# jinsungkim96/MPC-SensorlessAO

Hardware: AMD Instinct MI355X
Metric: MPC steps/sec (n=27, VAR(2), T=30) (higher is better)
Workload: dtype f64

## Files before the change

mpc-sensorlessao_amd/csrc/fmpc_affine.h:

```cpp
#pragma once
#include <hip/hip_runtime.h>
#include "fmpc_host.h"
#include "../../include/fastmpc.h"

#define FA_N 27

struct FaStep {
    const double* x0; const double* x0p; const double* nu0;
    double* zout; double* nuout; double* u0out; int* status; int* iters; double* step;
    int* need;
};

struct FaParams {
    int n, m, T, nb, has_xf, batch, rows, tiles, step_ld;
    int nu_rows, nu_tiles;
    int ldz;
    int tiles_used, wgs_per_group;
    const double* img;
    const double* imgE; const double* imgEp;
    const double* elin; const double* eplin;
    const double* dx0T;
    double e0, ep0, normE, norme, normEp, normep, rd2_0;
    const double* x0; const double* x0p; const double* nu0;
    double* zout; double* nuout; double* u0out; int* status; int* iters; double* step;
    int* need; int* handed;
    int* nflag;
    double* dump;
    int nsteps;
    FaStep steps[FMPC_STRETCH_MAX];
    int nlanes, wgs_per_lane;
    int lane_begin[FMPC_STRETCH_MAX + 1];
    const double* imgG;
    const int* plan;
    int jbase, nu_work;
    int nparts, nitems, swap;
};

#define FMPC_STRETCH_LANES_DEFAULT FMPC_STRETCH_MAX
hipError_t fmpc_launch_affine(FaParams P, int num_cu, hipStream_t stream, const unsigned* supersedes = nullptr);
hipError_t fmpc_launch_affine_nu(FaParams P, int grid, bool nt, hipStream_t stream);
```

mpc-sensorlessao_amd/csrc/fmpc_api.hip:

```cpp
#include <hip/hip_runtime.h>
#include <math.h>
#include <stdio.h>
#include <stdlib.h>
#include <string.h>
#include <atomic>
#include <map>
#include <mutex>
#include <new>
#include <vector>

#include "../../include/fastmpc.h"
#include "fmpc_device.h"
#include "fmpc_panel.h"
#include "fmpc_host.h"
#include "fmpc_first.h"
#include "fmpc_affine.h"
#include "fmpc_loopu0.h"
#include "fmpc_tiled.h"
#include "fmpc_rampcold.h"
#include "fmpc_bank.h"
#include "fmpc_records.h"
#include "fmpc_kkt.h"
#include "fmpc_estimator.h"
#include "fmpc_handle.h"
// ... 603 lines not shown
bool fmpc_capturing(hipStream_t stream) {
    hipStreamCaptureStatus st = hipStreamCaptureStatusNone;
    return hipStreamIsCapturing(stream, &st) == hipSuccess && st == hipStreamCaptureStatusActive;
}

struct FmpcChainStep {
    FaStep a;
    FwParams w;
    bool superseded;
    unsigned same_outputs;
};
struct FmpcStretch {
    fmpc_handle h = nullptr;
    int nsteps = 0;
    FaParams A;
    double k = 0.0; int n_newton = 0, zld = 0, g3 = 0; bool z_null = false, z_aligned = false;
    size_t wave_lds = 0, ws_stride = 0; int num_cu = 0;
    FwParams* table = nullptr;
    FmpcChainStep st[FMPC_STRETCH_MAX];
    size_t nodes_seen = 0;
};
static std::mutex fmpc_st_mu;
static std::map<hipStream_t, FmpcStretch> fmpc_st_map;
static std::atomic<int> fmpc_st_open{0};

static bool fmpc_capture_nodes(hipStream_t stream, size_t* count) {
    hipStreamCaptureStatus st = hipStreamCaptureStatusNone;
    unsigned long long id = 0; hipGraph_t graph = nullptr; const hipGraphNode_t* deps = nullptr; size_t ndeps = 0;
    if (hipStreamGetCaptureInfo_v2(stream, &st, &id, &graph, &deps, &ndeps) != hipSuccess || st != hipStreamCaptureStatusActive || !graph)
        return false;
    size_t n = 0;
    if (hipGraphGetNodes(graph, nullptr, &n) != hipSuccess) return false;
    *count = n;
    return true;
}
static void fmpc_stretch_look(FmpcStretch& S, hipStream_t stream) {
    size_t n = 0;
    S.nodes_seen = fmpc_capture_nodes(stream, &n) ? n : 0;
}
static bool fmpc_stretch_foreign(FmpcStretch& S, hipStream_t stream) {
    size_t n = 0;
    if (S.nsteps == 0 || !fmpc_capture_nodes(stream, &n) || n == S.nodes_seen) return false;
    S.nsteps = 0; S.h = nullptr;
    S.nodes_seen = n;
    return true;
}

static int fmpc_stretch_flush(FmpcStretch& S, hipStream_t stream) {
    if (S.nsteps == 0) return FMPC_OK;
    const int n = S.nsteps;
    fmpc_handle h = S.h;
    S.nsteps = 0; S.h = nullptr;
    if (!fmpc_capturing(stream) && h->ev && h->ev_valid && h->last_stream != stream && hipStreamWaitEvent(stream, h->ev, 0) != hipSuccess)
        return FMPC_E_HIP;
    FaParams A = S.A;
    A.nsteps = n;
    for (int i = 0; i < n; ++i) A.steps[i] = S.st[i].a;
    unsigned same[FMPC_STRETCH_MAX];
    for (int j = 0; j < n; ++j) {
        same[j] = S.st[j].same_outputs & ((1u << j) - 1u);
        for (int i = 0; i < j; ++i) if (same[j] >> i & 1u) same[j] |= same[i];
    }
    if (fmpc_launch_affine(A, S.num_cu, stream, same) != hipSuccess) return FMPC_E_HIP;
    int live[FMPC_STRETCH_MAX], nlive = 0;
    for (int i = 0; i < n; ++i) if (!S.st[i].superseded) live[nlive++] = i;
    int launches = 1;
    if (nlive == 1 || S.z_null) {
        for (int j = 0; j < nlive; ++j) {
            FwParams P = S.st[live[j]].w;
            if (j + 1 < nlive) { P.handed = nullptr; P.nflag = nullptr; }
            if (fmpc_launch_wave(P, S.g3, S.wave_lds, stream) != hipSuccess) return FMPC_E_HIP;
            ++launches;
        }
    } else {
        int g = S.num_cu / nlive;
        if (g > S.g3) g = S.g3;
        if (g < 1) return FMPC_E_UNSUPPORTED;
        FwChainStep T[FMPC_STRETCH_MAX];
        for (int j = 0; j < nlive; ++j) {
            const FwParams& P = S.st[live[j]].w;
            T[j] = {P.x0, P.x0p, P.nu0, P.zout, P.nuout, P.u0out, P.status, P.iters, P.step, P.list,
                    j + 1 == nlive ? P.handed : nullptr, P.ws + (size_t)j * g * fmpc_wave_waves_per_wg() * S.ws_stride};
        }
        if (fmpc_launch_wave_chain(S.st[live[0]].w, T, nlive, S.table, g, S.wave_lds, stream) != hipSuccess) return FMPC_E_HIP;
        launches += 2;
    }
    h->st_steps = n; h->st_launches = launches;
    if (!fmpc_capturing(stream) && h->ev && hipEventRecord(h->ev, stream) == hipSuccess) { h->ev_valid = 1; h->last_stream = stream; }
    fmpc_stretch_look(S, stream);
    return FMPC_OK;
}

static void fmpc_stretch_flush_handle_locked(fmpc_handle h, bool keep_one, hipStream_t keep);
static int fmpc_stretch_flush_stream(hipStream_t stream, fmpc_handle h = nullptr) {
    if (fmpc_st_open.load() == 0) return FMPC_OK;
    std::lock_guard<std::mutex> lk(fmpc_st_mu);
    if (h) fmpc_stretch_flush_handle_locked(h, true, stream);
    auto it = fmpc_st_map.find(stream);
    if (it == fmpc_st_map.end()) return FMPC_OK;
    if (fmpc_stretch_foreign(it->second, stream)) return FMPC_E_UNSUPPORTED;
    return fmpc_stretch_flush(it->second, stream);
}
static void fmpc_stretch_flush_handle_locked(fmpc_handle h, bool keep_one, hipStream_t keep) {
    for (auto& kv : fmpc_st_map)
        if (kv.second.nsteps && kv.second.h == h && !(keep_one && kv.first == keep) && !fmpc_stretch_foreign(kv.second, kv.first))
            (void)fmpc_stretch_flush(kv.second, kv.first);
}
static void fmpc_stretch_flush_handle(fmpc_handle h) {
    if (fmpc_st_open.load() == 0) return;
    std::lock_guard<std::mutex> lk(fmpc_st_mu);
    fmpc_stretch_flush_handle_locked(h, false, nullptr);
}

extern "C" int fmpc_stretch_begin(void* stream_) {
    hipStream_t stream = (hipStream_t)stream_;
    std::lock_guard<std::mutex> lk(fmpc_st_mu);
    if (fmpc_st_map.count(stream)) return FMPC_E_UNSUPPORTED;
    FmpcStretch& S = fmpc_st_map[stream];
    fmpc_stretch_look(S, stream);
    fmpc_st_open.fetch_add(1);
    return FMPC_OK;
}
extern "C" int fmpc_stretch_end(void* stream_) {
    hipStream_t stream = (hipStream_t)stream_;
    std::lock_guard<std::mutex> lk(fmpc_st_mu);
    auto it = fmpc_st_map.find(stream);
    if (it == fmpc_st_map.end()) return FMPC_E_UNSUPPORTED;
    int rc = FMPC_OK;
    if (it->second.nsteps) {
        if (it->second.h && hipSetDevice(it->second.h->device) != hipSuccess) rc = FMPC_E_HIP;
        else if (fmpc_stretch_foreign(it->second, stream)) rc = FMPC_E_UNSUPPORTED;
        else rc = fmpc_stretch_flush(it->second, stream);
    }
    fmpc_st_map.erase(it);
    fmpc_st_open.fetch_sub(1);
    return rc;
}
extern "C" int fmpc_last_stretch(fmpc_handle h, int* steps, int* launches) {
    if (!h) return FMPC_E_NULL;
    if (steps) *steps = h->st_steps.load();
    if (launches) *launches = h->st_launches.load();
    return FMPC_OK;
}

static inline bool fmpc_overlap(const void* a, size_t na, const void* b, size_t nb) {
    if (!a || !b || !na || !nb) return false;
    const char* pa = (const char*)a; const char* pb = (const char*)b;
    return pa < pb + nb && pb < pa + na;
}
struct FmpcStepRanges { const void* in[3]; size_t nin[3]; const void* out[6]; size_t nout[6]; };
static FmpcStepRanges fmpc_step_ranges(const FaParams& A, const FaStep& a) {
    FmpcStepRanges R;
    const size_t B = (size_t)A.batch, d = sizeof(double);
    R.in[0] = a.x0; R.nin[0] = B * A.n * d;
    R.in[1] = a.x0p; R.nin[1] = B * A.n * d;
    R.in[2] = a.nu0; R.nin[2] = B * A.nb * A.n * d;
    const size_t ldz = A.ldz > A.rows ? A.ldz : A.rows;
    R.out[0] = a.zout; R.nout[0] = ((B - 1) * ldz + A.rows) * d;
    R.out[1] = a.nuout; R.nout[1] = B * A.nb * A.n * d;
    R.out[2] = a.u0out; R.nout[2] = B * A.m * d;
    R.out[3] = a.status; R.nout[3] = B * sizeof(int);
    R.out[4] = a.iters; R.nout[4] = B * sizeof(int);
    R.out[5] = a.step; R.nout[5] = B * A.step_ld * d;
    return R;
}
static bool fmpc_stretch_accepts(const FmpcStretch& S, fmpc_handle h, const FmpcSolve& s, const FaStep& a, int zld, bool z_null, unsigned* supersedes) {
    *supersedes = 0;
    if (S.h != h || S.nsteps >= FMPC_STRETCH_MAX || memcmp(&S.k, &s.k, sizeof(double)) != 0 || S.A.batch != s.batch) return false;
    if (S.n_newton != s.n_newton || S.zld != zld || S.z_null != z_null || S.z_aligned != (((size_t)a.zout & 127) == 0)) return false;
    const FaStep& f = S.st[0].a;
    if ((f.nuout == nullptr) != (a.nuout == nullptr) || (f.u0out == nullptr) != (a.u0out == nullptr) || (f.status == nullptr) != (a.status == nullptr) ||
        (f.iters == nullptr) != (a.iters == nullptr) || (f.step == nullptr) != (a.step == nullptr)) return false;
    const FmpcStepRanges N = fmpc_step_ranges(S.A, a);
    for (int i = 0; i < S.nsteps; ++i) {
        const FaStep& b = S.st[i].a;
        const FmpcStepRanges O = fmpc_step_ranges(S.A, b);
        for (int x = 0; x < 3; ++x)
            for (int y = 0; y < 6; ++y)
                if (fmpc_overlap(N.in[x], N.nin[x], O.out[y], O.nout[y]) || fmpc_overlap(O.in[x], O.nin[x], N.out[y], N.nout[y])) return false;
        if (a.zout == b.zout && a.nuout == b.nuout && a.u0out == b.u0out && a.status == b.status && a.iters == b.iters && a.step == b.step) {
            *supersedes |= 1u << i;
            continue;
        }
        for (int x = 0; x < 6; ++x)
            for (int y = 0; y < 6; ++y)
                if (fmpc_overlap(N.out[x], N.nout[x], O.out[y], O.nout[y])) return false;
    }
    return true;
}

static int fmpc_stretch_settle(fmpc_handle h, hipStream_t stream) {
    if (!h->st_cur || h->st_cur->nsteps == 0) return FMPC_OK;
    return fmpc_stretch_flush(*h->st_cur, stream);
}
static int fmpc_guard_begin_queued(fmpc_handle h, hipStream_t stream) {
    if (fmpc_capturing(stream)) return FMPC_OK;
    if (!h->ev && hipEventCreateWithFlags(&h->ev, hipEventDisableTiming) != hipSuccess) return FMPC_E_HIP;
    if (h->ev_valid && stream != h->last_stream && hipStreamWaitEvent(stream, h->ev, 0) != hipSuccess) return FMPC_E_HIP;
    return FMPC_OK;
}
int fmpc_guard_begin(fmpc_handle h, hipStream_t stream) {
    const int rcs = fmpc_stretch_flush_stream(stream, h);
    if (rcs != FMPC_OK) return rcs;
    if (fmpc_capturing(stream)) return FMPC_OK;
    if (!h->ev && hipEventCreateWithFlags(&h->ev, hipEventDisableTiming) != hipSuccess) return FMPC_E_HIP;
    if (h->ev_valid && stream != h->last_stream && hipStreamWaitEvent(stream, h->ev, 0) != hipSuccess) return FMPC_E_HIP;
    return FMPC_OK;
}
void fmpc_guard_end(fmpc_handle h, hipStream_t stream) {
    if (fmpc_capturing(stream)) return;
    if (h->ev && hipEventRecord(h->ev, stream) == hipSuccess) { h->ev_valid = 1; h->last_stream = stream; }
}

static void fmpc_panel_params(fmpc_handle h, double k, FpParams& Q) {
    memset(&Q, 0, sizeof(Q));
    Q.m = h->m; Q.mp = h->pn_mp; Q.T = h->T; Q.nb = h->nb; Q.has_xf = h->has_xf; Q.var2 = h->var_order == 2 ? 1 : 0;
    Q.simg = h->pn_pool + h->pn_o_simg; Q.limg = h->pn_pool + h->pn_o_limg;
    Q.sched_f = h->pn_sched; Q.sched_b = h->pn_sched + (size_t)FP_MAX_STEPS(h->nb) * FP_STEP_INTS; Q.nsf = h->pn_nsf; Q.nsb = h->pn_nsb;
    Q.btimg = h->pn_pool + h->pn_o_bt; Q.aimg = h->pn_pool + h->pn_o_aimg;
    Q.vec = h->pn_pool + h->pn_o_vec; Q.ucon = h->pn_pool + h->pn_o_ucon;
    Q.rd2_0 = h->pn_rd2_0; Q.rp2c = h->pn_rp2c; Q.dump = h->pn_pool + h->pn_o_dump;
    Q.dzimg = h->pn_pool + h->pn_o_dz; Q.dzimg_len = h->pn_dz_len;
    Q.kbar = k;
    Q.jimg = h->inv_jimg; Q.nuc = h->inv_nuc; Q.jks = h->inv_jks; Q.jksp = 16 * ((h->inv_jks + 15) / 16 + 3); Q.eimg = h->inv_eimg;
    Q.jst = h->inv_jst; Q.nucst = h->inv_nucst; Q.gate_only = 0;
    Q.gw = nullptr; Q.gwn = h->T * h->n;
}

static int fmpc_build_inverse(fmpc_handle h, double k, hipStream_t stream) {
    const int n = h->n, T = h->T, nb = h->nb, TN = T * n, nrow = nb * n;
    const int ncol = 2 * n + TN, np = 1 + ncol + 2 * n, npanels = (np + FP_NP - 1) / FP_NP;
    const double scale = FMPC_INV_SCALE;
    h->inv_valid = 0;
    std::vector<double> hx0((size_t)np * n, 0.0), hx0p((size_t)np * n, 0.0), hw((size_t)np * TN, 0.0);
    for (int j = 0; j < n; ++j) { hx0[(size_t)(1 + j) * n + j] = scale; hx0p[(size_t)(1 + n + j) * n + j] = scale; }
    for (int j = 0; j < TN; ++j) hw[(size_t)(1 + 2 * n + j) * TN + j] = scale;
    for (int j = 0; j < n; ++j)
        for (int e = 0; e < TN; ++e) {
            hw[(size_t)(1 + ncol + j) * TN + e] = -scale * h->hm_m1[(size_t)e * n + j];
            hw[(size_t)(1 + ncol + n + j) * TN + e] = -scale * h->hm_m2[(size_t)e * n + j];
        }
    DevBuf<double> d;
    const size_t o_x0 = 0, o_x0p = o_x0 + hx0.size(), o_w = o_x0p + hx0p.size(), o_gate = o_w + hw.size(),
                 o_nu = o_gate + 2 * (size_t)np, total = o_nu + (size_t)npanels * nrow * FP_NP;
    int rc = d.alloc(total, stream);
    if (rc != FMPC_OK) return rc;
    std::vector<double> nu((size_t)npanels * nrow * FP_NP);
    if (hipMemcpyAsync(d + o_x0, hx0.data(), hx0.size() * sizeof(double), hipMemcpyHostToDevice, stream) != hipSuccess ||
        hipMemcpyAsync(d + o_x0p, hx0p.data(), hx0p.size() * sizeof(double), hipMemcpyHostToDevice, stream) != hipSuccess ||
        hipMemcpyAsync(d + o_w, hw.data(), hw.size() * sizeof(double), hipMemcpyHostToDevice, stream) != hipSuccess) rc = FMPC_E_HIP;
    if (rc == FMPC_OK) {
        FpParams Q;
        fmpc_panel_params(h, k, Q);
        Q.batch = np; Q.npanels = npanels; Q.step_ld = 1;
        Q.x0 = d + o_x0; Q.x0p = d + o_x0p; Q.w = d + o_w; Q.nu0 = nullptr;
        Q.nuws = d + o_nu; Q.gate = d + o_gate; Q.handed = nullptr;
        const int pgrid = npanels < h->num_cu ? npanels : h->num_cu;
        if (fmpc_launch_panel(Q, pgrid, fmpc_panel_lds_used(h->nb, h->pn_mp, h->pn_nsf + h->pn_nsb), stream) != hipSuccess ||
            hipMemcpyAsync(nu.data(), d + o_nu, nu.size() * sizeof(double), hipMemcpyDeviceToHost, stream) != hipSuccess ||
            hipStreamSynchronize(stream) != hipSuccess) rc = FMPC_E_HIP;
    }
    d.release();
    if (rc != FMPC_OK) return rc;
    std::vector<double> img, nuc, jst, ncs, img2, eimg, J4, nuc4;
    const bool finite = fmpc_host_inverse_images(n, T, nb, h->var_order == 2, h->inv_jks, h->inv_jks2, h->hm_a1.data(), h->hm_a2.data(), nu,
                                                 img, nuc, jst, ncs, img2, eimg, J4, nuc4);
    if (!jst.empty() &&
        (hipMemcpy(h->inv_jst, jst.data(), jst.size() * sizeof(double), hipMemcpyHostToDevice) != hipSuccess ||
         hipMemcpy(h->inv_nucst, ncs.data(), ncs.size() * sizeof(double), hipMemcpyHostToDevice) != hipSuccess)) return FMPC_E_HIP;
    if (!finite) return FMPC_OK;
    if (hipMemcpy(h->inv_jimg2, img2.data(), img2.size() * sizeof(double), hipMemcpyHostToDevice) != hipSuccess) return FMPC_E_HIP;
    if (hipMemcpy(h->inv_eimg, eimg.data(), eimg.size() * sizeof(double), hipMemcpyHostToDevice) != hipSuccess ||
        hipMemcpy(h->inv_jimg, img.data(), img.size() * sizeof(double), hipMemcpyHostToDevice) != hipSuccess ||
        hipMemcpy(h->inv_nuc, nuc.data(), nuc.size() * sizeof(double), hipMemcpyHostToDevice) != hipSuccess) return FMPC_E_HIP;
    h->hm_J4.swap(J4); h->hm_nuc.swap(nuc4);
    h->hm_J4_valid = 1; h->hm_J4_k = k; h->fm_valid = 0;
    h->inv_valid = 1; h->inv_k = k;
    return FMPC_OK;
}

static int fmpc_build_first_move(fmpc_handle h, double k, hipStream_t stream) {
    h->fm_valid = 0;
    if (!h->hm_J4_valid || h->hm_J4_k != k) return FMPC_E_UNSUPPORTED;
    const int n = h->n, m = h->m, T = h->T, TN = T * n;
    FmpcFirstIn In;
    In.n = n; In.m = m; In.T = T; In.nb = h->nb; In.var2 = h->var_order == 2 ? 1 : 0; In.has_xf = h->has_xf;
    In.bt = h->hm_bt.data(); In.umax = h->hm_umax.data(); In.umin = h->hm_umin.data(); In.umid = h->hm_umid.data();
    In.xmid = h->hm_xmid.data(); In.R2 = h->hm_R2.data(); In.rl = h->hm_rl.data(); In.a1 = h->hm_a1.data(); In.a2 = h->hm_a2.data();
    In.m1 = h->hm_m1.data(); In.m2 = h->hm_m2.data(); In.xf = h->hm_xf.empty() ? h->hm_xmid.data() : h->hm_xf.data();
    In.J = h->hm_J4.data(); In.nuc = h->hm_nuc.data(); In.k = k;
    FmpcFirstOut O;
    fmpc_host_build_first_move(In, O);
    for (double v : O.K0t) if (!std::isfinite(v)) return FMPC_E_UNSUPPORTED;
    for (double v : O.E) if (!std::isfinite(v)) return FMPC_E_UNSUPPORTED;
    std::vector<double> pool;
    auto push = [&](const std::vector<double>& v) { const size_t o = pool.size(); pool.insert(pool.end(), v.begin(), v.end()); while (pool.size() % 2) pool.push_back(0.0); return o; };
    std::vector<double> m12t((size_t)2 * n * TN), dx0T(n);
    for (int e = 0; e < TN; ++e)
        for (int q = 0; q < n; ++q) { m12t[(size_t)q * TN + e] = h->hm_m1[(size_t)e * n + q]; m12t[(size_t)(n + q) * TN + e] = h->hm_m2[(size_t)e * n + q]; }
    for (int r = 0; r < n; ++r) dx0T[r] = h->hm_Qf2[r] * h->hm_xmid[r] + h->hm_qfl[r];
    const size_t oK = push(O.K0t), ou = push(O.u0c), oE = push(O.Ec), oe = push(O.e), oEp = push(O.Epc), oep = push(O.ep), om = push(m12t), od = push(dx0T);
    h->fa_valid = 0;
    FmpcAffineOut AO;
    size_t oA = 0, oAE = 0, oAEp = 0, oAl = 0, oAlp = 0, oAd = 0, oAG = 0, oAP = 0;
    bool fa_ok = !h->fa_disabled && 2 * n + 2 <= FA_KC;
    if (fa_ok) {
        FmpcAffineIn AI;
        AI.n = n; AI.m = m; AI.T = T; AI.nb = h->nb; AI.has_xf = h->has_xf; AI.ncJ = 4 * n;
        AI.bt = In.bt; AI.umax = In.umax; AI.umin = In.umin; AI.umid = In.umid; AI.xmid = In.xmid; AI.R2 = In.R2; AI.rl = In.rl;
        AI.Q2 = h->hm_Q2.data(); AI.Qf2 = h->hm_Qf2.data(); AI.ql = h->hm_ql.data(); AI.qfl = h->hm_qfl.data(); AI.a1 = In.a1; AI.a2 = In.a2;
        AI.J = In.J; AI.nuc = In.nuc; AI.k = k;
        fmpc_host_build_affine(AI, AO);
        for (double v : AO.img) if (!std::isfinite(v)) { fa_ok = false; break; }
    }
    if (fa_ok) {
        const int nc = 4 * n, nd = 2 * n;
        std::vector<double> E64((size_t)64 * FA_KC, 0.0), Ep64((size_t)64 * FA_KC, 0.0), el(64, 0.0), epl(64, 0.0), imgE, imgEp;
        for (int r = 0; r < nd; ++r) {
            for (int c = 0; c < nd; ++c) { E64[(size_t)r * FA_KC + c] = O.E[(size_t)r * nc + c]; Ep64[(size_t)r * FA_KC + c] = O.Ep[(size_t)r * nc + c]; }
            el[r] = 2.0 * O.e[r]; epl[r] = -2.0 * O.ep[r];
        }
        fmpc_host_mfma_a_images(E64.data(), 64, imgE);
        fmpc_host_mfma_a_images(Ep64.data(), 64, imgEp);
        oA = push(AO.img); oAE = push(imgE); oAEp = push(imgEp); oAl = push(el); oAlp = push(epl);
        oAd = push(std::vector<double>(4096, 0.0));
        if (!AO.imgG.empty()) {
            std::vector<double> planw((AO.plan.size() * sizeof(FmpcNuStage) + sizeof(double) - 1) / sizeof(double), 0.0);
            memcpy(planw.data(), AO.plan.data(), AO.plan.size() * sizeof(FmpcNuStage));
            oAG = push(AO.imgG); oAP = push(planw);
        }
    }
    h->fl_valid = 0; h->fs_valid = 0;
    size_t oLU = 0, oLE = 0, oLEp = 0, oSU = 0, oSE = 0, oSEp = 0, oSB = 0;
    const bool fl_ok = !h->fl_disabled && 4 * n + 1 <= 4 * FL_KS;
    const bool fs_ok = fl_ok && !h->fs_disabled && n == 27 && m <= 144;
    if (fl_ok) {
        FmpcLoopImages LI;
        fmpc_host_build_loop_images(O, n, m, FL_KS, false, nullptr, LI);
        oLU = push(LI.imgU); oLE = push(LI.imgE); oLEp = push(LI.imgEp);
    }
    if (fs_ok) {
        FmpcLoopImages LI;
        fmpc_host_build_loop_images(O, n, m, FL_KS, true, In.bt, LI);
        oSU = push(LI.imgU); oSE = push(LI.imgE); oSEp = push(LI.imgEp); oSB = push(LI.imgB);
    }
    const int rc = h->fm_pool.assign(pool.data(), pool.size(), stream);
    if (rc != FMPC_OK) return rc;
    FmParams& P = h->fm_P;
    memset(&P, 0, sizeof(P));
    P.n = n; P.m = m; P.T = T; P.nb = h->nb; P.var2 = In.var2; P.has_xf = h->has_xf;
    P.bt = h->dev.Bt; P.K0t = h->fm_pool + oK; P.u0c = h->fm_pool + ou; P.E = h->fm_pool + oE; P.e = h->fm_pool + oe;
    P.Ep = h->fm_pool + oEp; P.ep = h->fm_pool + oep; P.m12t = h->fm_pool + om; P.dx0T = h->fm_pool + od;
    P.e0 = O.e0; P.ep0 = O.ep0; P.normE = O.normE; P.norme = O.norme; P.normEp = O.normEp; P.normep = O.normep; P.rd2_0 = h->pn_rd2_0;
    h->fm_valid = 1; h->fm_k = k;
    if (fa_ok) {
        FaParams& A = h->fa_P;
        memset(&A, 0, sizeof(A));
        A.n = n; A.m = m; A.T = T; A.nb = h->nb; A.has_xf = h->has_xf; A.rows = AO.rows; A.tiles = AO.tiles; A.nu_rows = AO.nu_rows; A.nu_tiles = AO.nu_tiles;
        A.img = h->fm_pool + oA; A.imgE = h->fm_pool + oAE; A.imgEp = h->fm_pool + oAEp; A.elin = h->fm_pool + oAl; A.eplin = h->fm_pool + oAlp; A.dump = h->fm_pool + oAd;
        if (!AO.imgG.empty()) {
            A.imgG = h->fm_pool + oAG; A.plan = (const int*)(h->fm_pool + oAP); A.jbase = AO.jbase; A.nu_work = fmpc_host_nu_work(AO.plan);
        }
        A.dx0T = P.dx0T; A.e0 = O.e0; A.ep0 = O.ep0; A.normE = O.normE; A.norme = O.norme; A.normEp = O.normEp; A.normep = O.normep; A.rd2_0 = h->pn_rd2_0;
        h->fa_valid = 1;
    }
    if (fl_ok) {
        FlParams& L = h->fl_P;
        memset(&L, 0, sizeof(L));
        L.n = n; L.m = m; L.T = T; L.nb = h->nb; L.has_xf = h->has_xf; L.var2 = In.var2;
        L.imgU = h->fm_pool + oLU; L.imgE = h->fm_pool + oLE; L.imgEp = h->fm_pool + oLEp;
        L.dx0T = P.dx0T; L.e0 = O.e0; L.ep0 = O.ep0; L.normE = O.normE; L.norme = O.norme; L.normEp = O.normEp; L.normep = O.normep; L.rd2_0 = h->pn_rd2_0;
        h->fl_valid = 1;
        if (fs_ok) {
            h->fs_P = L;
            h->fs_P.imgU = h->fm_pool + oSU; h->fs_P.imgE = h->fm_pool + oSE; h->fs_P.imgEp = h->fm_pool + oSEp;
            memset(&h->fs_I, 0, sizeof(h->fs_I));
            const int Tn = T * n;
            h->fs_I.rs = (Tn + 63) / 64; h->fs_I.rows = (Tn + h->fs_I.rs - 1) / h->fs_I.rs;
            h->fs_I.imgB = h->fm_pool + oSB; h->fs_I.M1 = h->loop_M1; h->fs_I.M2 = h->loop_M2;
            h->fs_valid = 1;
        }
    }
    return FMPC_OK;
}

static int fmpc_ensure_wave_ws(fmpc_handle h, size_t* stride_out, hipStream_t stream) {
    const int wpw = fmpc_wave_waves_per_wg();
    const size_t stride = fmpc_wave_ws_doubles(h->n, h->m, h->wave.mp, h->T, h->nb);
    const int rc = h->ws.grow(stride * (size_t)h->num_cu * wpw, stream);
    if (rc != FMPC_OK) return rc;
    *stride_out = stride;
    return FMPC_OK;
}

static FwParams fmpc_wave_params(fmpc_handle h, const FmpcSolve& s, size_t stride, int zld = 0) {
    FwParams P;
    memset(&P, 0, sizeof(P));
    P.M = h->dev; P.V = h->wave;
    P.batch = s.batch; P.max_iter = fmpc_max_iter(s); P.step_ld = fmpc_step_ld(s.n_newton); P.kbar = s.k;
    P.x0 = s.x0; P.x0p = s.x0_pre; P.w = s.w; P.zinit = s.z_init; P.nu0 = s.nu0;
    P.zout = s.z_out; P.nuout = s.nu_out; P.status = s.status; P.iters = s.iters; P.step = s.step; P.u0out = s.u0_out;
    P.zld = zld > 0 ? zld : h->T * (h->n + h->m);
    P.ws = h->ws; P.ws_stride = stride;
    P.sh_fac = h->sh_fac; P.sh_rs = h->sh_rs; P.sh_ok = h->sh_ok; P.cold = h->cold_d;
    return P;
}

static int fmpc_wave_grid(fmpc_handle h, int batch) {
    const int wpw = fmpc_wave_waves_per_wg();
    const int grid = (batch + wpw - 1) / wpw;
    return grid < h->num_cu ? grid : h->num_cu;
}

static int fmpc_launch_flagged(fmpc_handle h, const FmpcSolve& s, int grid, size_t stride, int* need, int* nflag = nullptr, int zld = 0) {
    FwParams P = fmpc_wave_params(h, s, stride, zld);
    P.mode = FW_MODE_SHARED; P.handed = h->pn_cnt; P.pphase = 3; P.list = need; P.nflag = nflag;
    return fmpc_launch_wave(P, grid, h->wave_lds, s.stream) == hipSuccess ? FMPC_OK : FMPC_E_HIP;
}

static int fmpc_ensure_cold(fmpc_handle h, double k, size_t stride, hipStream_t stream) {
    if (h->sh_valid && h->sh_k == k) return FMPC_OK;
    if (h->sh_valid && hipStreamSynchronize(stream) != hipSuccess) return FMPC_E_HIP;
    double* scr = h->sh_scratch;
    const FmpcSolve one = {1, scr, scr, nullptr, nullptr, nullptr, 1, k, scr + ((h->n + 15) & ~15), nullptr, nullptr, nullptr, nullptr,
                           nullptr, stream, 0};
    FwParams P = fmpc_wave_params(h, one, stride);
    P.mode = FW_MODE_EXPORT;
    if (fmpc_launch_wave(P, 1, h->wave_lds, stream) != hipSuccess) return FMPC_E_HIP;
    if (fmpc_upload_cold(h, k, stream) != FMPC_OK) return FMPC_E_HIP;
    if (h->pn_enabled && fmpc_upload_panel(h, k, stream) != FMPC_OK) return FMPC_E_HIP;
    h->sh_valid = 1; h->sh_k = k;
    return FMPC_OK;
}

int fmpc_scratch_z(fmpc_handle h, int batch, hipStream_t stream) {
    return h->zs.grow((size_t)batch * h->T * (h->n + h->m), stream);
}


static int fmpc_path_tiled(fmpc_handle h, const FmpcSolve& s) {
    const int t_ = h->prec == FMPC_PREC_F32_MIXED ? 1 : 0;
    const int few = (!t_ && !h->denseR && h->n <= 31 && h->n != FP_N && s.batch <= 512 && !h->force_tiled) ? 4 : 0;
    return fmpc_solve_tiled(h, t_, s, few);
}

static int fmpc_path_generic(fmpc_handle h, const FmpcSolve& s) {
    h->last_path = FMPC_PATH_GENERIC;
    const int grid = fmpc_grid_for(h, s.batch);
    size_t stride = 0;
    const int rc = fmpc_ensure_ws(h, h->generic_big ? grid : h->num_cu * h->wg_per_cu, &stride, s.stream);
    if (rc != FMPC_OK) return rc;
    hipError_t e = fmpc_launch_generic(h->dev, s.batch, grid, s.x0, s.x0_pre, s.w, s.z_init, s.nu0, fmpc_max_iter(s), s.k,
                                       s.z_out, s.nu_out, s.status, s.iters, s.step, fmpc_step_ld(s.n_newton),
                                       h->ws, stride, s.stream, h->generic_big);
    if (e == hipSuccess && s.u0_out)
        e = fmpc_launch_unpack(h->n, h->m, h->T, s.batch, s.z_out, nullptr, nullptr, s.u0_out, s.stream);
    return e == hipSuccess ? FMPC_OK : FMPC_E_HIP;
}

static int fmpc_path_affine(fmpc_handle h, const FmpcSolve& s, size_t stride, int zld, bool z_null) {
    if (!h->fm_valid || h->fm_k != s.k) {
        { const int rcq = fmpc_stretch_settle(h, s.stream); if (rcq != FMPC_OK) return rcq; }
        if (hipStreamSynchronize(s.stream) != hipSuccess) return FMPC_E_HIP;
        const int rcf = fmpc_build_first_move(h, s.k, s.stream);
        if (rcf != FMPC_OK && rcf != FMPC_E_UNSUPPORTED) return rcf;
    }
    if (!(h->fm_valid && h->fm_k == s.k && h->fa_valid)) return FMPC_E_UNSUPPORTED;
    if ((size_t)s.batch > h->fa_need_cap) {
        { const int rcq = fmpc_stretch_settle(h, s.stream); if (rcq != FMPC_OK) return rcq; }
        size_t cap = 256;
        while (cap < (size_t)s.batch) cap *= 2;
        h->fa_need_cap = 0;
        const int rc = h->fa_need.alloc((size_t)FMPC_STRETCH_MAX * cap, s.stream);
        if (rc != FMPC_OK) return rc;
        h->fa_need_cap = cap;
    }
    FaParams A = h->fa_P;
    A.batch = s.batch; A.step_ld = fmpc_step_ld(s.n_newton);
    A.x0 = s.x0; A.x0p = s.x0_pre; A.nu0 = s.nu0; A.zout = z_null ? nullptr : s.z_out; A.nuout = s.nu_out; A.u0out = s.u0_out;
    A.status = s.status; A.iters = s.iters; A.step = s.step; A.need = h->fa_need; A.handed = h->pn_cnt;
    int* const nf = h->fa_nflag;
    static const bool no_nflag = [] { const char* e = getenv("FMPC_NO_NFLAG"); return e && e[0] == '1'; }();
    A.nflag = no_nflag ? nullptr : nf;
    A.ldz = zld;
    A.nsteps = 0;
    const int grid = fmpc_wave_grid(h, s.batch);
    const int g3 = grid < 64 ? grid : 64;
    if (h->st_cur) {
        FmpcStretch& S = *h->st_cur;
        FaStep a = {A.x0, A.x0p, A.nu0, A.zout, A.nuout, A.u0out, A.status, A.iters, A.step, nullptr};
        unsigned sup = 0;
        if (S.nsteps > 0 && !fmpc_stretch_accepts(S, h, s, a, zld, z_null, &sup)) { const int rcq = fmpc_stretch_settle(h, s.stream); if (rcq != FMPC_OK) return rcq; }
        const int i = S.nsteps;
        a.need = h->fa_need + (size_t)i * h->fa_need_cap;
        if (i == 0) {
            S.h = h; S.A = A; S.k = s.k; S.n_newton = s.n_newton; S.zld = zld; S.z_null = z_null; S.z_aligned = ((size_t)A.zout & 127) == 0;
            S.g3 = g3; S.wave_lds = h->wave_lds; S.ws_stride = stride; S.num_cu = h->num_cu; S.table = (FwParams*)h->fw_chain.p;
            fmpc_stretch_look(S, s.stream);
            sup = 0;
        }
        for (int j = 0; j < i; ++j) if (sup & (1u << j)) S.st[j].superseded = true;
        S.st[i].a = a;
        S.st[i].superseded = false;
        S.st[i].same_outputs = sup;
        FwParams W = fmpc_wave_params(h, s, stride, zld);
        W.mode = FW_MODE_SHARED; W.handed = h->pn_cnt; W.pphase = 3; W.list = a.need; W.nflag = no_nflag ? nullptr : nf;
        S.st[i].w = W;
        S.nsteps = i + 1;
        h->last_path = FMPC_PATH_PANEL; h->pn_split_last = 0; h->inv_last = 2;
        return FMPC_OK;
    }
    if (fmpc_launch_affine(A, h->num_cu, s.stream) != hipSuccess) return FMPC_E_HIP;
    const int rc = fmpc_launch_flagged(h, s, g3, stride, h->fa_need, no_nflag ? nullptr : nf, zld);
    h->last_path = FMPC_PATH_PANEL; h->pn_split_last = 0; h->inv_last = 2;
    return rc;
}

static int fmpc_path_panel(fmpc_handle h, const FmpcSolve& s, size_t stride, int zld, bool z_null) {
    const int batch = s.batch, max_iter = fmpc_max_iter(s);
    const int npanels = (batch + FP_NP - 1) / FP_NP;
    if ((size_t)batch > h->pn_cap) {
        { const int rcq = fmpc_stretch_settle(h, s.stream); if (rcq != FMPC_OK) return rcq; }
        h->pn_cap = 0;
        if (h->pn_gate.alloc((size_t)batch * 2, s.stream) != FMPC_OK ||
            h->pn_epsp.alloc((size_t)npanels * h->T * FP_NP, s.stream) != FMPC_OK ||
            h->pn_rnp.alloc((size_t)npanels * h->T * FP_NP, s.stream) != FMPC_OK ||
            h->pn_list.alloc((size_t)batch, s.stream) != FMPC_OK ||
            h->pn_nuws.alloc((size_t)npanels * FP_NP * h->nb * h->n, s.stream) != FMPC_OK) return FMPC_E_ALLOC;
        h->pn_cap = batch;
    }
    const bool lowrank = h->lp_hint && s.w != nullptr && h->lp_v != nullptr;
    const bool dense_form = h->inv_enabled && (s.w == nullptr || lowrank || batch <= h->inv_max_batch);
    if (dense_form && (!h->inv_valid || h->inv_k != s.k) && !(h->inv_failed && h->inv_failed_k == s.k)) {
        { const int rcq = fmpc_stretch_settle(h, s.stream); if (rcq != FMPC_OK) return rcq; }
        if (hipStreamSynchronize(s.stream) != hipSuccess) return FMPC_E_HIP;
        const int rcb = fmpc_build_inverse(h, s.k, s.stream);
        if (rcb != FMPC_OK) return rcb;
        h->inv_failed = h->inv_valid ? 0 : 1; h->inv_failed_k = s.k;
    }
    if (dense_form && h->inv_valid && s.w == nullptr && max_iter == 1 && (s.nu_out == nullptr || !z_null) && !h->fa_disabled && h->n == FP_N) {
        const int rca = fmpc_path_affine(h, s, stride, zld, z_null);
        if (rca != FMPC_E_UNSUPPORTED) return rca;
    }
    if (zld) return FMPC_E_UNSUPPORTED;
    { const int rcq = fmpc_stretch_settle(h, s.stream); if (rcq != FMPC_OK) return rcq; }
    FpParams Q;
    fmpc_panel_params(h, s.k, Q);
    Q.batch = batch; Q.npanels = npanels; Q.step_ld = fmpc_step_ld(s.n_newton);
    Q.x0 = s.x0; Q.x0p = s.x0_pre; Q.w = s.w; Q.nu0 = s.nu0;
    Q.zout = s.z_out; Q.status = s.status; Q.iters = s.iters; Q.step = s.step;
    Q.nuws = h->pn_nuws; Q.nuout = s.nu_out;
    Q.gate = h->pn_gate; Q.epsp = h->pn_epsp; Q.handed = h->pn_cnt;
    Q.rnp = h->pn_rnp;
    const int split = max_iter > 1;
    const int pgrid = npanels < h->num_cu ? npanels : h->num_cu;
    h->inv_last = dense_form && h->inv_valid;
    const bool fuse = h->inv_last && h->inv_fuse && s.w == nullptr && !h->has_xf && max_iter == 1;
    Q.gate_only = fuse ? 1 : 0;
    const bool u0only = z_null && max_iter == 1 && s.nu_out == nullptr;
    Q.u0out = s.u0_out;
    if (h->inv_last) {
        if (lowrank) { Q.gw = h->lp_v; Q.gwn = 2 * h->n; Q.jimg = h->inv_jimg2; Q.jks = h->inv_jks2; Q.jksp = 16 * ((h->inv_jks2 + 15) / 16 + 3); }
        else { Q.gw = s.w; Q.gwn = h->T * h->n; }
    }
    hipError_t e;
    if (h->inv_last) e = fmpc_launch_inv(Q, s.stream);
    else e = fmpc_launch_panel(Q, pgrid, fmpc_panel_lds_used(h->nb, h->pn_mp, h->pn_nsf + h->pn_nsb), s.stream);
    if (e != hipSuccess) return FMPC_E_HIP;
    const int ppx = (npanels + 7) / 8;
    const int dgrid = 8 * ((ppx * h->T + FD_WAVES - 1) / FD_WAVES);
    e = fmpc_launch_dz(Q, dgrid, split, s.stream, fuse ? 1 : 0, u0only ? 1 : 0);
    if (e != hipSuccess) return FMPC_E_HIP;
    const int grid = fmpc_wave_grid(h, batch);
    for (int ph = split ? 1 : 0; ph <= (split ? 2 : 0); ++ph) {
        int g2 = grid;
        if (ph == 2) {
            const int last = ((volatile int*)h->pn_cnt_host.p)[1];
            if (last >= 0) {
                const int wpw2 = fmpc_wave_waves_per_wg();
                int want = (last + last / 2 + wpw2 - 1) / wpw2 + 4;
                if (want < 8) want = 8;
                if (want < g2) g2 = want;
            }
        }
        if (ph == 2 && h->small_tiled) {
            const int last = ((volatile int*)h->pn_cnt_host.p)[1];
            const int hint = last >= 0 ? last + last / 2 + 16 : 0;
            const int rc_t = fmpc_solve_tiled(h, 0, s, h->small_nw, h->pn_list, h->pn_cnt + 1, h->pn_nuws, hint);
            if (rc_t == FMPC_OK) continue;
            if (rc_t != FMPC_E_UNSUPPORTED && rc_t != FMPC_E_ALLOC) return rc_t;
        }
        FwParams P = fmpc_wave_params(h, s, stride);
        P.mode = FW_MODE_SHARED; P.gate = h->pn_gate; P.epsp = h->pn_epsp; P.handed = h->pn_cnt; P.nuws = h->pn_nuws;
        P.pphase = ph; P.rnp = h->pn_rnp; P.list = h->pn_list; P.u0_done = u0only ? 1 : 0;
        e = fmpc_launch_wave(P, g2, h->wave_lds, s.stream);
        if (e != hipSuccess) return FMPC_E_HIP;
    }
    if (split && hipMemcpyAsync(h->pn_cnt_host, h->pn_cnt, 2 * sizeof(int), hipMemcpyDeviceToHost, s.stream) != hipSuccess)
        return FMPC_E_HIP;
    h->last_path = FMPC_PATH_PANEL; h->pn_split_last = split;
    return e == hipSuccess ? FMPC_OK : FMPC_E_HIP;
}

static int fmpc_path_small_tiled(fmpc_handle h, const FmpcSolve& s) {
    return fmpc_solve_tiled(h, 0, s, s.batch <= 512 ? h->small_nw : 2);
}

static int fmpc_path_split(fmpc_handle h, const FmpcSolve& s, size_t stride) {
    const int last = h->gn_cnt_host ? ((volatile int*)h->gn_cnt_host.p)[1] : -1;
    const int gn_hint = last >= 0 ? last + last / 2 + 16 : 0;
    FmpcTiledPlan gplan;
    if (fmpc_tiled_plan(h, 0, s.batch, s.stream, h->small_nw, gn_hint, &gplan) != FMPC_OK) return FMPC_E_UNSUPPORTED;
    const size_t nbn = (size_t)h->nb * h->n;
    if ((size_t)s.batch > h->gn_cap) {
        h->gn_cap = 0;
        if (h->gn_list.alloc((size_t)s.batch, s.stream) != FMPC_OK || h->gn_cnt.alloc(2, s.stream) != FMPC_OK ||
            h->gn_nu.alloc((size_t)s.batch * nbn, s.stream) != FMPC_OK) return FMPC_E_ALLOC;
        h->gn_cap = s.batch;
    }
    if (!h->gn_cnt_host) {
        if (h->gn_cnt_host.alloc(2, s.stream) != FMPC_OK) return FMPC_E_ALLOC;
        h->gn_cnt_host[0] = -1; h->gn_cnt_host[1] = -1;
    }
    double* nu_arr = s.nu_out ? s.nu_out : h->gn_nu;
    hipLaunchKernelGGL(fmpc_zero_ints, dim3(1), dim3(64), 0, s.stream, h->gn_cnt, 2);
    if (hipGetLastError() != hipSuccess) return FMPC_E_HIP;
    FwParams P = fmpc_wave_params(h, s, stride);
    P.nuout = nu_arr; P.handed = h->gn_cnt; P.pphase = 4; P.list = h->gn_list;
    if (fmpc_launch_wave(P, fmpc_wave_grid(h, s.batch), h->wave_lds, s.stream) != hipSuccess) return FMPC_E_HIP;
    h->last_path = FMPC_PATH_WAVE;
    FmpcSolve c = s;
    c.z_init = nullptr; c.nu_out = nu_arr;
    const int rc_t = fmpc_solve_tiled(h, 0, c, h->small_nw, h->gn_list, h->gn_cnt + 1, nullptr, gn_hint, &gplan);
    if (rc_t != FMPC_OK) return rc_t;
    if (hipMemcpyAsync(h->gn_cnt_host, h->gn_cnt, 2 * sizeof(int), hipMemcpyDeviceToHost, s.stream) != hipSuccess) return FMPC_E_HIP;
    return FMPC_OK;
}

static int fmpc_path_wave(fmpc_handle h, const FmpcSolve& s, int mode, size_t stride) {
    FwParams P = fmpc_wave_params(h, s, stride);
    P.mode = mode;
    const hipError_t e = fmpc_launch_wave(P, fmpc_wave_grid(h, s.batch), h->wave_lds, s.stream);
    h->last_path = mode == FW_MODE_SHARED ? FMPC_PATH_SHARED : FMPC_PATH_WAVE;
    return e == hipSuccess ? FMPC_OK : FMPC_E_HIP;
}

static int fmpc_solve_device_inner(fmpc_handle h, FmpcSolve s) {
    if (!h || !s.x0 || (!s.z_out && !s.u0_out)) return FMPC_E_NULL;
    if (s.batch < 0) return FMPC_E_DIM;
    if (s.batch == 0) return FMPC_OK;
    const int max_iter = fmpc_max_iter(s);
    const bool z_null = s.z_out == nullptr;
    if (z_null) {
        if ((size_t)s.batch * h->T * (h->n + h->m) > h->zs.cap) { const int rcq = fmpc_stretch_settle(h, s.stream); if (rcq != FMPC_OK) return rcq; }
        const int rcz = fmpc_scratch_z(h, s.batch, s.stream);
        if (rcz != FMPC_OK) return rcz;
        s.z_out = h->zs;
    }
    const int zld = (!z_null && s.ldz > h->T * (h->n + h->m)) ? s.ldz : 0;
    if (zld && (s.w != nullptr || s.z_init != nullptr || max_iter != 1 || h->prec == FMPC_PREC_F32_MIXED || h->force_tiled || h->denseQ ||
                h->denseR || !h->use_wave || !h->sh_enabled || !h->pn_enabled)) return FMPC_E_UNSUPPORTED;
    if (h->prec == FMPC_PREC_F32_MIXED || h->force_tiled || ((h->denseQ || h->denseR) && !h->generic_big) ||
        (!h->use_wave && (!h->generic_ok || h->prefer_tiled))) {
        { const int rcq = fmpc_stretch_settle(h, s.stream); if (rcq != FMPC_OK) return rcq; }
// ... 952 lines not shown
```

mpc-sensorlessao_amd/csrc/fmpc_host.cpp:

```cpp
#include "fmpc_host.h"
#include "fmpc_bank.h"
#include "../../include/fastmpc.h"
#include "fmpc_noise.h"

#include <algorithm>
#include <math.h>
#include <stdio.h>
#include <stdlib.h>

bool fmpc_host_is_diag(const double* M, int n) {
    for (int c = 0; c < n; ++c)
        for (int r = 0; r < n; ++r)
            if (r != c && fmpc_host_cm(M, n, r, c) != 0.0) return false;
    return true;
}

bool fmpc_host_spd_inverse(const std::vector<double>& A, int n, std::vector<double>& inv) {
    typedef long double ld;
    std::vector<ld> L((size_t)n * n, 0.0L), Li((size_t)n * n, 0.0L);
    for (int c = 0; c < n; ++c) {
        ld d = A[c * n + c];
        for (int k = 0; k < c; ++k) d -= L[c * n + k] * L[c * n + k];
        if (!(d > 0.0L)) return false;
        const ld l = sqrtl(d);
// ... 592 lines not shown
            dz[D.UC + mp + j] = uc[mp + j]; dz[D.UC + 2 * mp + j] = uc[2 * mp + j]; dz[D.UC + 3 * mp + j] = uc[3 * mp + j];
        }
        for (int j = 0; j < mp; ++j) {
            const bool in = j < m;
            dz[D.UX + j] = in ? In.R2[j] * In.umid[j] + In.rl[j] : 0.0;
            dz[D.UX + mp + j] = in ? In.R2[j] : 0.0;
            dz[D.UX + 2 * mp + j] = in ? In.umax[j] - In.umid[j] : 1.0;
            dz[D.UX + 3 * mp + j] = in ? In.umid[j] - In.umin[j] : 1.0;
        }
        for (int r = 0; r < 32; ++r) {
            dz[D.XQ + r] = vec[V.xc + r]; dz[D.XQ + 32 + r] = vec[V.xc + (T - 1) * 32 + r];
            dz[D.XQ + 64 + r] = vec[V.iq + r]; dz[D.XQ + 96 + r] = vec[V.iq + (T - 1) * 32 + r];
        }
    }
    Out.valid = 1;
    Out.nimg = nimg;
    return 0;
}


void fmpc_host_build_first_move(const FmpcFirstIn& In, FmpcFirstOut& Out) {
    typedef long double ld;
    const int n = In.n, m = In.m, T = In.T, nb = In.nb, nc = 4 * n;
    const bool var2 = In.var2 != 0;
    Out.nc = nc;
    std::vector<double> cu(m), wc(m), av(m);
    for (int j = 0; j < m; ++j) {
        const double sp = In.umax[j] - In.umid[j], sm = In.umid[j] - In.umin[j];
        const double dp = 1.0 / sp, dm = 1.0 / sm;
        const double hc = In.k * (dp * dp + dm * dm);
        cu[j] = In.R2[j] * In.umid[j] + In.rl[j] + In.k * (dp - dm);
        wc[j] = 1.0 / (In.R2[j] + hc);
        av[j] = hc * wc[j];
    }
    const double* bt = In.bt;
    Out.K0t.assign((size_t)nc * m, 0.0); Out.u0c.assign(m, 0.0);
    for (int j = 0; j < m; ++j) {
        ld t = 0.0L;
        for (int r = 0; r < n; ++r) t += (ld)bt[(size_t)j * n + r] * (ld)In.nuc[r];
        Out.u0c[j] = (double)((ld)In.umid[j] + (ld)wc[j] * (t - (ld)cu[j]));
        for (int c = 0; c < nc; ++c) {
            ld s = 0.0L;
            for (int r = 0; r < n; ++r) s += (ld)bt[(size_t)j * n + r] * (ld)In.J[(size_t)r * nc + c];
            Out.K0t[(size_t)c * m + j] = (double)((ld)wc[j] * s);
        }
    }
    std::vector<ld> Ma2((size_t)n * n, 0.0L);
    for (int r = 0; r < n; ++r)
        for (int q = 0; q < n; ++q) {
            ld t = 0.0L;
            for (int j = 0; j < m; ++j) t += (ld)bt[(size_t)j * n + r] * (ld)av[j] * (ld)av[j] * (ld)bt[(size_t)j * n + q];
            Ma2[(size_t)r * n + q] = t;
        }
    std::vector<ld> E((size_t)nc * nc, 0.0L), e(nc, 0.0L), tmp((size_t)n * nc), bg(n), g(m);
    ld e0 = 0.0L;
    for (int s = 0; s < T; ++s) {
        const double* Js = In.J + (size_t)s * n * nc;
        const double* ncs = In.nuc + (size_t)s * n;
        for (int j = 0; j < m; ++j) {
            ld t = 0.0L;
            for (int r = 0; r < n; ++r) t += (ld)bt[(size_t)j * n + r] * (ld)ncs[r];
            g[j] = (ld)av[j] * (t - (ld)cu[j]);
            e0 += g[j] * g[j];
        }
        for (int r = 0; r < n; ++r) {
            ld t = 0.0L;
            for (int j = 0; j < m; ++j) t += (ld)bt[(size_t)j * n + r] * (ld)av[j] * g[j];
            bg[r] = t;
        }
        for (int r = 0; r < n; ++r)
            for (int c = 0; c < nc; ++c) {
                ld t = 0.0L;
                for (int q = 0; q < n; ++q) t += Ma2[(size_t)r * n + q] * (ld)Js[(size_t)q * nc + c];
                tmp[(size_t)r * nc + c] = t;
            }
        for (int c1 = 0; c1 < nc; ++c1) {
            ld t = 0.0L;
            for (int r = 0; r < n; ++r) t += (ld)Js[(size_t)r * nc + c1] * bg[r];
            e[c1] += t;
            for (int c2 = 0; c2 < nc; ++c2) {
                ld u = 0.0L;
                for (int r = 0; r < n; ++r) u += (ld)Js[(size_t)r * nc + c1] * tmp[(size_t)r * nc + c2];
                E[(size_t)c1 * nc + c2] += u;
            }
        }
    }
    std::vector<ld> Ep((size_t)nc * nc, 0.0L), ep(nc, 0.0L), row(nc);
    ld ep0 = 0.0L;
    std::vector<ld> bu(n, 0.0L), a1x(n, 0.0L), a2x(n, 0.0L);
    for (int r = 0; r < n; ++r) {
        for (int j = 0; j < m; ++j) bu[r] += (ld)bt[(size_t)j * n + r] * (ld)In.umid[j];
        for (int q = 0; q < n; ++q) { a1x[r] += (ld)In.a1[r * n + q] * (ld)In.xmid[q]; a2x[r] += (ld)In.a2[r * n + q] * (ld)In.xmid[q]; }
    }
    for (int i = 0; i < nb; ++i)
        for (int r = 0; r < n; ++r) {
            ld cp;
            for (int c = 0; c < nc; ++c) row[c] = 0.0L;
            if (i < T) {
                cp = (ld)In.xmid[r] - bu[r] - (i >= 1 ? a1x[r] : 0.0L) - (i >= 2 ? a2x[r] : 0.0L);
                if (i == 0) for (int q = 0; q < n; ++q) { row[q] = In.a1[r * n + q]; row[n + q] = var2 ? (ld)In.a2[r * n + q] : 0.0L; }
                if (i == 1 && var2) for (int q = 0; q < n; ++q) row[q] = In.a2[r * n + q];
                for (int q = 0; q < n; ++q) {
                    row[2 * n + q] = -(ld)In.m1[((size_t)i * n + r) * n + q];
                    row[3 * n + q] = -(ld)In.m2[((size_t)i * n + r) * n + q];
                }
            } else {
                cp = (ld)In.xmid[r] - (ld)In.xf[r];
            }
            ep0 += cp * cp;
            for (int c1 = 0; c1 < nc; ++c1) {
                if (row[c1] == 0.0L) continue;
                ep[c1] += row[c1] * cp;
                for (int c2 = 0; c2 < nc; ++c2) Ep[(size_t)c1 * nc + c2] += row[c1] * row[c2];
            }
        }
    auto fro = [](const std::vector<ld>& v) { ld s = 0.0L; for (ld x : v) s += x * x; return (double)sqrtl(s); };
    Out.E.resize(E.size()); Out.Ep.resize(Ep.size()); Out.e.resize(nc); Out.ep.resize(nc);
    for (size_t i = 0; i < E.size(); ++i) { Out.E[i] = (double)E[i]; Out.Ep[i] = (double)Ep[i]; }
    for (int c = 0; c < nc; ++c) { Out.e[c] = (double)e[c]; Out.ep[c] = (double)ep[c]; }
    Out.e0 = (double)e0; Out.ep0 = (double)ep0;
    const int H = nc / 2 + 1;
    Out.Ec.assign((size_t)H * nc, 0.0); Out.Epc.assign((size_t)H * nc, 0.0);
    for (int j = 0; j < H; ++j)
        for (int r = 0; r < nc; ++r) {
            const int c = (r + j) % nc;
            const ld wgt = j == 0 ? 1.0L : ((j == nc / 2 && r >= nc / 2) ? 0.0L : 2.0L);
            const ld se = (E[(size_t)r * nc + c] + E[(size_t)c * nc + r]) * 0.5L, sp = (Ep[(size_t)r * nc + c] + Ep[(size_t)c * nc + r]) * 0.5L;
            Out.Ec[(size_t)j * nc + r] = (double)(wgt * se);
            Out.Epc[(size_t)j * nc + r] = (double)(wgt * sp);
        }
    Out.normE = fro(E); Out.norme = fro(e); Out.normEp = fro(Ep); Out.normep = fro(ep);
}

void fmpc_host_mfma_images(const double* M, int rows, int cols, int ks, std::vector<double>& img) {
    const int tiles = (rows + 15) / 16;
    img.assign((size_t)tiles * ks * 64, 0.0);
    for (int t = 0; t < tiles; ++t)
        for (int q = 0; q < ks; ++q)
            for (int g = 0; g < 4; ++g)
                for (int r = 0; r < 16; ++r) {
                    const int row = 16 * t + r, col = 4 * q + g;
                    if (row < rows && col < cols) img[((size_t)t * ks + q) * 64 + g * 16 + r] = M[(size_t)row * cols + col];
                }
}

void fmpc_host_build_loop_images(const FmpcFirstOut& O, int n, int m, int ks, bool fused, const double* bt, FmpcLoopImages& out) {
    const int nc = 4 * n, kc = 4 * ks, cst = fused ? kc - 1 : nc;
    auto col = [&](int c) { return fused ? ks * (c / n) + c % n : c; };
    std::vector<double> U((size_t)m * kc, 0.0), E2((size_t)kc * kc, 0.0), Ep2((size_t)kc * kc, 0.0);
    for (int j = 0; j < m; ++j) {
        for (int c = 0; c < nc; ++c) U[(size_t)j * kc + col(c)] = O.K0t[(size_t)c * m + j];
        U[(size_t)j * kc + cst] = O.u0c[j];
    }
    for (int r = 0; r < nc; ++r) {
        const int rr = col(r);
        for (int c = 0; c < nc; ++c) {
            const int cc = col(c);
            const double wgt = cc / 16 > rr / 16 ? 2.0 : (cc / 16 == rr / 16 ? 1.0 : 0.0);
            E2[(size_t)rr * kc + cc] = wgt * O.E[(size_t)r * nc + c];
            Ep2[(size_t)rr * kc + cc] = wgt * O.Ep[(size_t)r * nc + c];
        }
        E2[(size_t)rr * kc + cst] = 2.0 * O.e[r];
        Ep2[(size_t)rr * kc + cst] = -2.0 * O.ep[r];
    }
    fmpc_host_mfma_images(U.data(), m, kc, ks, out.imgU);
    fmpc_host_mfma_images(E2.data(), kc, kc, ks, out.imgE);
    fmpc_host_mfma_images(Ep2.data(), kc, kc, ks, out.imgEp);
    out.imgB.clear();
    if (fused && bt) {
        std::vector<double> Brm((size_t)n * m);
        for (int q = 0; q < n; ++q)
            for (int c = 0; c < m; ++c) Brm[(size_t)q * m + c] = bt[(size_t)c * n + q];
        fmpc_host_mfma_images(Brm.data(), n, m, (m + 3) / 4, out.imgB);
    }
}

void fmpc_host_mfma_a_images(const double* M, int rows, std::vector<double>& img) {
    const int tiles = (rows + 15) / 16;
    img.assign((size_t)tiles * FA_KS * 64, 0.0);
    for (int t = 0; t < tiles; ++t)
        for (int q = 0; q < FA_KS; ++q)
            for (int g = 0; g < 4; ++g)
                for (int r = 0; r < 16; ++r) {
                    const int row = 16 * t + r;
                    if (row < rows) img[((size_t)t * FA_KS + q) * 64 + g * 16 + r] = M[(size_t)row * FA_KC + 4 * q + g];
                }
}

void fmpc_host_build_affine(const FmpcAffineIn& In, FmpcAffineOut& Out) {
    typedef long double ld;
    const int n = In.n, m = In.m, T = In.T, s = n + m, nd = 2 * n, ncJ = In.ncJ;
    Out.rows = T * s; Out.tiles = (Out.rows + 15) / 16;
    Out.Kz.assign((size_t)Out.rows * FA_KC, 0.0);
    std::vector<ld> cu(m), wc(m);
    for (int j = 0; j < m; ++j) {
        const ld sp = (ld)In.umax[j] - (ld)In.umid[j], sm = (ld)In.umid[j] - (ld)In.umin[j];
        const ld dp = 1.0L / sp, dm = 1.0L / sm;
        cu[j] = (ld)In.R2[j] * (ld)In.umid[j] + (ld)In.rl[j] + (ld)In.k * (dp - dm);
        wc[j] = 1.0L / ((ld)In.R2[j] + (ld)In.k * (dp * dp + dm * dm));
    }
    auto nuv = [&](int blk, int r, int c) -> ld {
        return c < nd ? (ld)In.J[((size_t)blk * n + r) * ncJ + c] : (ld)In.nuc[(size_t)blk * n + r];
    };
    for (int st = 0; st < T; ++st) {
        for (int j = 0; j < m; ++j) {
            double* row = &Out.Kz[((size_t)st * s + j) * FA_KC];
            for (int c = 0; c <= nd; ++c) {
                ld t = 0.0L;
                for (int r = 0; r < n; ++r) t += (ld)In.bt[(size_t)j * n + r] * nuv(st, r, c);
                if (c == nd) t = (ld)In.umid[j] + wc[j] * (t - cu[j]); else t *= wc[j];
                row[c] = (double)t;
            }
        }
        const int jx = st + 1;
        const bool last = jx == T;
        for (int r = 0; r < n; ++r) {
            double* row = &Out.Kz[((size_t)st * s + m + r) * FA_KC];
            const ld q2 = last ? (ld)In.Qf2[r] : (ld)In.Q2[r], ql = last ? (ld)In.qfl[r] : (ld)In.ql[r];
            for (int c = 0; c <= nd; ++c) {
                ld v = -nuv(jx - 1, r, c);
                if (jx < T) for (int q = 0; q < n; ++q) v += (ld)In.a1[q * n + r] * nuv(jx, q, c);
                if (jx + 1 < T) for (int q = 0; q < n; ++q) v += (ld)In.a2[q * n + r] * nuv(jx + 1, q, c);
                if (last && In.has_xf) v -= nuv(T, r, c);
                if (c == nd) v = (ld)In.xmid[r] + (v - (q2 * (ld)In.xmid[r] + ql)) / q2; else v /= q2;
                row[c] = (double)v;
            }
        }
    }
    fmpc_host_mfma_a_images(Out.Kz.data(), Out.rows, Out.img);
    Out.nu_rows = In.nb * n; Out.nu_tiles = (Out.nu_rows + 15) / 16;
    std::vector<double> Jn((size_t)Out.nu_rows * FA_KC, 0.0), imgn;
    for (int r = 0; r < Out.nu_rows; ++r) {
        for (int c = 0; c < nd; ++c) Jn[(size_t)r * FA_KC + c] = In.J[(size_t)r * ncJ + c];
        Jn[(size_t)r * FA_KC + nd] = In.nuc[r];
    }
    fmpc_host_mfma_a_images(Jn.data(), Out.nu_rows, imgn);
    Out.img.insert(Out.img.end(), imgn.begin(), imgn.end());
    Out.jbase = Out.tiles + Out.nu_tiles;
    fmpc_host_plan_nu(m, n, T, Out.plan);
    if (n != 27) { Out.imgG.clear(); return; }
    std::vector<double> Jp((size_t)32 * FA_KC);
    for (int st = 1; st < T; ++st) {
        std::fill(Jp.begin(), Jp.end(), 0.0);
        for (int r = 0; r < n; ++r) {
            for (int c = 0; c < nd; ++c) Jp[(size_t)r * FA_KC + c] = In.J[((size_t)st * n + r) * ncJ + c];
            Jp[(size_t)r * FA_KC + nd] = In.nuc[(size_t)st * n + r];
        }
        Jp[(size_t)n * FA_KC + nd] = 1.0;
        fmpc_host_mfma_a_images(Jp.data(), 32, imgn);
        Out.img.insert(Out.img.end(), imgn.begin(), imgn.end());
    }
    int nut = 0;
    for (int st = 0; st < T; ++st) nut += Out.plan[st].nu;
    Out.imgG.assign((size_t)nut * FA_NU_KS * 64, 0.0);
    for (int st = 1; st < T; ++st)
        for (int u = 0; u < Out.plan[st].nu; ++u) {
            double* im = &Out.imgG[(size_t)(Out.plan[st].ub + u) * FA_NU_KS * 64];
            for (int r = 0; r < 16; ++r) {
                const int j = 16 * (Out.plan[st].tb + u) + r - st * s;
                for (int c = 0; c <= n; ++c) {
                    const ld v = c < n ? wc[j] * (ld)In.bt[(size_t)j * n + c] : (ld)In.umid[j] - wc[j] * cu[j];
                    im[(size_t)(c >> 2) * 64 + (c & 3) * 16 + r] = (double)v;
                }
            }
        }
}

void fmpc_host_plan_nu(int m, int n, int T, std::vector<FmpcNuStage>& plan) {
    const int s = n + m, tiles = (T * s + 15) / 16;
    plan.assign(T > 0 ? T : 0, FmpcNuStage{0, 0, 0, 0});
    int ub = 0;
    for (int j = 0; j < T; ++j) {
        const int tb = (s * j + 15) / 16;
        int te = (s * (j + 1) + 15) / 16;
        if (te > tiles) te = tiles;
        int nu = j >= 1 ? (s * j + m) / 16 - tb : 0;
        if (nu < 0) nu = 0;
        if (nu > te - tb) nu = te - tb;
        plan[j] = FmpcNuStage{tb, nu, te - tb - nu, ub};
        ub += nu;
    }
}

int fmpc_host_nu_work(const std::vector<FmpcNuStage>& plan) {
    int work = 0;
    for (const FmpcNuStage& S : plan) work += 7 * S.nu + 14 * S.nd;
    return work;
}

int fmpc_host_nu_parts(int T, int work, int W) {
    if (T < 1 || W < 1) return 1;
    int bestP = 1; double best = -1.0;
    for (int P = 1; P <= 8; ++P) {
        const double cost = (double)((T * P + W - 1) / W) * (28.0 + (double)work / ((double)T * P));
        if (best < 0.0 || cost < best) { best = cost; bestP = P; }
    }
    return bestP;
}

int fmpc_host_nu_swap(int T, int parts, int W) {
    return parts == 1 && W >= 1 && T > W - 1 && T % W != 0 ? W - 1 : 0;
}

extern "C" int fmpc_debug_plan_nu(int m, int n, int T, int W, int* plan4, int* parts, int* swap) {
    if (m < 1 || n < 1 || T < 1 || !plan4) return -1;
    std::vector<FmpcNuStage> plan;
    fmpc_host_plan_nu(m, n, T, plan);
    for (int j = 0; j < T; ++j) { plan4[4 * j] = plan[j].tb; plan4[4 * j + 1] = plan[j].nu; plan4[4 * j + 2] = plan[j].nd; plan4[4 * j + 3] = plan[j].ub; }
    const int np = fmpc_host_nu_parts(T, fmpc_host_nu_work(plan), W);
    if (parts) *parts = np;
    if (swap) *swap = fmpc_host_nu_swap(T, np, W);
    return 0;
}
extern "C" int fmpc_debug_nu_cut(int cnt, int p, int parts, int* b, int* e) {
    if (cnt < 0 || parts < 1 || p < 0 || p >= parts || !b || !e) return -1;
    *b = FMPC_NU_CUT(cnt, p, parts); *e = FMPC_NU_CUT(cnt, p + 1, parts);
    return 0;
}
extern "C" int fmpc_debug_build_affine_nu(int n, int m, int T, int nb, int has_xf, double k, const double* const* arr, double* Kz, double* imgJ, double* imgG) {
    if (n != 27 || m < 1 || T < 1 || nb < T || !arr) return -1;
    FmpcAffineIn In;
    In.n = n; In.m = m; In.T = T; In.nb = nb; In.has_xf = has_xf; In.ncJ = 2 * n; In.k = k;
    In.bt = arr[0]; In.umax = arr[1]; In.umin = arr[2]; In.umid = arr[3]; In.xmid = arr[4]; In.R2 = arr[5]; In.rl = arr[6]; In.Q2 = arr[7];
    In.Qf2 = arr[8]; In.ql = arr[9]; In.qfl = arr[10]; In.a1 = arr[11]; In.a2 = arr[12]; In.J = arr[13]; In.nuc = arr[14];
    FmpcAffineOut Out;
    fmpc_host_build_affine(In, Out);
    if (Kz) std::copy(Out.Kz.begin(), Out.Kz.end(), Kz);
    if (imgJ) std::copy(Out.img.begin() + (size_t)Out.jbase * FA_KS * 64, Out.img.end(), imgJ);
    if (imgG) std::copy(Out.imgG.begin(), Out.imgG.end(), imgG);
    return (int)(Out.imgG.size() / (FA_NU_KS * 64));
}

void fmpc_host_build_ramp_cold(const FmpcRampColdIn& In, FmpcRampColdOut& Out) {
    typedef long double ld;
    const int n = In.n, m = In.m, T = In.T, nb = In.nb, s = n + m, Nz = T * s, nbn = nb * n;
    const bool var2 = In.var2 != 0, has_xf = In.has_xf != 0;
    Out.valid = 0;
    std::vector<ld> hb(m), gb(m), erb(m), grb(m);
    for (int c = 0; c < m; ++c) {
        const ld dp = 1.0L / ((ld)In.umax[c] - (ld)In.umid[c]), dm = 1.0L / ((ld)In.umid[c] - (ld)In.umin[c]);
        hb[c] = (ld)In.k * (dp * dp + dm * dm); gb[c] = (ld)In.k * (dp - dm);
        const ld rp = 1.0L / (ld)In.dumax[c], rm = 1.0L / (-(ld)In.dumin[c]);
        erb[c] = (ld)In.k * (rp * rp + rm * rm); grb[c] = (ld)In.k * (rp - rm);
    }
    Out.g0.assign((size_t)T * m, 0.0); Out.Gf.assign((size_t)T * T * m, 0.0); Out.hd.assign((size_t)T * m, 0.0);
    Out.erb.resize(m);
    std::vector<ld> Gl((size_t)T * T * m);
    std::vector<ld> dg(T), lo(T);
    for (int c = 0; c < m; ++c) {
        Out.erb[c] = (double)erb[c];
        for (int j = 0; j < T; ++j) {
            const ld hdj = hb[c] + (j >= 1 ? erb[c] : 0.0L) + (j + 1 < T ? erb[c] : 0.0L);
            Out.hd[(size_t)j * m + c] = (double)hdj;
            ld d = (ld)In.R2[c] + hdj;
            if (j > 0) d -= lo[j - 1] * lo[j - 1] * dg[j - 1];
            if (!(d > 0.0L) || !std::isfinite((double)d)) return;
            dg[j] = d;
            lo[j] = j + 1 < T ? -erb[c] / d : 0.0L;
        }
        for (int col = 0; col < T; ++col) {
            std::vector<ld> x(T, 0.0L);
            x[col] = 1.0L;
            for (int j = 1; j < T; ++j) x[j] -= lo[j - 1] * x[j - 1];
            for (int j = 0; j < T; ++j) x[j] /= dg[j];
            for (int j = T - 2; j >= 0; --j) x[j] -= lo[j] * x[j + 1];
            for (int j = 0; j < T; ++j) Gl[((size_t)j * T + col) * m + c] = x[j];
        }
        for (int i = 0; i < T; ++i)
            for (int j = 0; j < T; ++j) {
                const ld v = 0.5L * (Gl[((size_t)i * T + j) * m + c] + Gl[((size_t)j * T + i) * m + c]);
                Out.Gf[((size_t)i * T + j) * m + c] = (double)v;
            }
        for (int j = 0; j < T; ++j) Out.g0[(size_t)j * m + c] = Out.Gf[((size_t)j * T + 0) * m + c];
    }
    for (size_t i = 0; i < Gl.size(); ++i) Gl[i] = (ld)Out.Gf[i];
    auto qinv = [&](int jx, int r) -> ld { return 1.0L / (jx == T ? (ld)In.Qf2[r] : (ld)In.Q2[r]); };
    Out.gbar_u.assign((size_t)T * m, 0.0); Out.gbar_x.assign((size_t)T * n, 0.0);
    Out.phib_u.assign((size_t)T * m, 0.0); Out.phib_x.assign((size_t)T * n, 0.0);
    std::vector<ld> gu((size_t)T * m), gx((size_t)T * n), pu((size_t)T * m), px((size_t)T * n);
    for (int j = 0; j < T; ++j) {
        for (int c = 0; c < m; ++c)
            gu[(size_t)j * m + c] = (ld)In.R2[c] * (ld)In.umid[c] + (ld)In.rl[c] + gb[c] + (j >= 1 ? grb[c] : 0.0L) - (j + 1 < T ? grb[c] : 0.0L);
        for (int r = 0; r < n; ++r) {
            const bool last = j + 1 == T;
            gx[(size_t)j * n + r] = last ? (ld)In.Qf2[r] * (ld)In.xmid[r] + (ld)In.qfl[r] : (ld)In.Q2[r] * (ld)In.xmid[r] + (ld)In.ql[r];
        }
    }
    for (int j = 0; j < T; ++j) {
        for (int c = 0; c < m; ++c) {
            ld t = 0.0L;
            for (int i = 0; i < T; ++i) t -= Gl[((size_t)j * T + i) * m + c] * gu[(size_t)i * m + c];
            pu[(size_t)j * m + c] = t;
        }
        for (int r = 0; r < n; ++r) px[(size_t)j * n + r] = -gx[(size_t)j * n + r] * qinv(j + 1, r);
    }
    for (size_t i = 0; i < gu.size(); ++i) { Out.gbar_u[i] = (double)gu[i]; Out.phib_u[i] = (double)pu[i]; }
    for (size_t i = 0; i < gx.size(); ++i) { Out.gbar_x[i] = (double)gx[i]; Out.phib_x[i] = (double)px[i]; }
    struct Ent { int col; ld v; };
    std::vector<std::vector<Ent>> Cr(nbn);
    for (int i = 0; i < T; ++i)
        for (int r = 0; r < n; ++r) {
            std::vector<Ent>& row = Cr[(size_t)i * n + r];
            row.push_back({i * s + m + r, 1.0L});
            for (int c = 0; c < m; ++c) row.push_back({i * s + c, -(ld)In.bt[(size_t)c * n + r]});
            if (i >= 1) for (int q = 0; q < n; ++q) row.push_back({(i - 1) * s + m + q, -(ld)In.a1[(size_t)r * n + q]});
            if (var2 && i >= 2) for (int q = 0; q < n; ++q) row.push_back({(i - 2) * s + m + q, -(ld)In.a2[(size_t)r * n + q]});
        }
    if (has_xf) for (int r = 0; r < n; ++r) Cr[(size_t)T * n + r].push_back({(T - 1) * s + m + r, 1.0L});
    auto zstart = [&](int col) -> ld { const int e = col % s; return e < m ? (ld)In.umid[e] : (ld)In.xmid[e - m]; };
    Out.cpb.assign(nbn, 0.0); Out.betab.assign(nbn, 0.0);
    auto phib_at = [&](int col) -> ld { const int j = col / s, e = col % s; return e < m ? pu[(size_t)j * m + e] : px[(size_t)j * n + (e - m)]; };
    std::vector<ld> cpl(nbn), betal(nbn);
    for (int a = 0; a < nbn; ++a) {
        ld cz = 0.0L, cp = 0.0L;
        for (const Ent& e : Cr[a]) { cz += e.v * zstart(e.col); cp += e.v * phib_at(e.col); }
        if (a >= T * n) cz -= (ld)In.xf[a - T * n];
        cpl[a] = cz; betal[a] = cp + cz;
        Out.cpb[a] = (double)cz; Out.betab[a] = (double)(cp + cz);
    }
    std::vector<ld> P((size_t)Nz * nbn, 0.0L);
    for (int b = 0; b < nbn; ++b)
        for (const Ent& e : Cr[b]) {
            const int j = e.col / s, el = e.col % s;
            if (el < m) { for (int jj = 0; jj < T; ++jj) P[((size_t)jj * s + el) * nbn + b] += Gl[((size_t)jj * T + j) * m + el] * e.v; }
            else P[(size_t)e.col * nbn + b] += e.v * qinv(j + 1, el - m);
        }
    std::vector<ld> Y((size_t)nbn * nbn, 0.0L);
    for (int a = 0; a < nbn; ++a)
        for (const Ent& e : Cr[a]) {
            const ld* prow = &P[(size_t)e.col * nbn];
            ld* yrow = &Y[(size_t)a * nbn];
            for (int b = 0; b < nbn; ++b) yrow[b] += e.v * prow[b];
        }
    for (int j = 0; j < nbn; ++j) {
        ld d = Y[(size_t)j * nbn + j];
        for (int q = 0; q < j; ++q) d -= Y[(size_t)j * nbn + q] * Y[(size_t)j * nbn + q];
        if (!(d > 0.0L) || !std::isfinite((double)d)) return;
        const ld l = sqrtl(d);
        Y[(size_t)j * nbn + j] = l;
        for (int i = j + 1; i < nbn; ++i) {
            ld v = Y[(size_t)i * nbn + j];
            for (int q = 0; q < j; ++q) v -= Y[(size_t)i * nbn + q] * Y[(size_t)j * nbn + q];
            Y[(size_t)i * nbn + j] = v / l;
        }
    }
    std::vector<ld> Yi((size_t)nbn * nbn, 0.0L), x(nbn);
    for (int col = 0; col < nbn; ++col) {
        for (int i = 0; i < nbn; ++i) {
            ld v = i == col ? 1.0L : 0.0L;
            if (i < col) { x[i] = 0.0L; continue; }
            for (int q = col; q < i; ++q) v -= Y[(size_t)i * nbn + q] * x[q];
            x[i] = v / Y[(size_t)i * nbn + i];
        }
        for (int i = nbn - 1; i >= 0; --i) {
            ld v = x[i];
            for (int q = i + 1; q < nbn; ++q) v -= Y[(size_t)q * nbn + i] * x[q];
            x[i] = v / Y[(size_t)i * nbn + i];
        }
        for (int i = 0; i < nbn; ++i) Yi[(size_t)i * nbn + col] = x[i];
    }
    const int ldy = (nbn + 1) & ~1;
    Out.Yinv.assign((size_t)nbn * ldy, 0.0);
    for (int a = 0; a < nbn; ++a)
        for (int b = 0; b < nbn; ++b) Out.Yinv[(size_t)a * ldy + b] = (double)(0.5L * (Yi[(size_t)a * nbn + b] + Yi[(size_t)b * nbn + a]));
    for (int a = 0; a < nbn; ++a)
        for (int b = 0; b < nbn; ++b) Yi[(size_t)a * nbn + b] = (ld)Out.Yinv[(size_t)a * ldy + b];
    std::vector<ld> Xi((size_t)m * nbn, 0.0L);
    for (int r = 0; r < m; ++r)
        for (int a = 0; a < nbn; ++a) {
            const ld pv = P[(size_t)r * nbn + a];
            if (pv == 0.0L) continue;
            for (int b = 0; b < nbn; ++b) Xi[(size_t)r * nbn + b] += pv * Yi[(size_t)a * nbn + b];
        }
    const int ldg = (m + 1) & ~1;
    Out.Xiu0t.assign((size_t)T * n * ldg, 0.0);
    for (int col = 0; col < T * n; ++col)
        for (int r = 0; r < m; ++r) Out.Xiu0t[(size_t)col * ldg + r] = (double)Xi[(size_t)r * nbn + col];
    Out.G.assign((size_t)m * ldg, 0.0);
    for (int r = 0; r < m; ++r)
        for (int c = r; c < m; ++c) {
            ld v = r == c ? Gl[((size_t)0 * T + 0) * m + r] : 0.0L;
            for (int b = 0; b < nbn; ++b) v -= Xi[(size_t)r * nbn + b] * P[(size_t)c * nbn + b];
            Out.G[(size_t)r * ldg + c] = (double)v; Out.G[(size_t)c * ldg + r] = (double)v;
        }
    Out.y0c.assign(m, 0.0);
    {
        std::vector<ld> nu(nbn, 0.0L);
        for (int a = 0; a < nbn; ++a) { ld v = 0.0L; for (int b = 0; b < nbn; ++b) v += Yi[(size_t)a * nbn + b] * betal[b]; nu[a] = v; }
        for (int r = 0; r < m; ++r) {
            ld v = pu[r];
            for (int b = 0; b < nbn; ++b) v -= P[(size_t)r * nbn + b] * nu[b];
            Out.y0c[r] = (double)v;
        }
    }
    for (double v : Out.Yinv) if (!std::isfinite(v)) return;
    for (double v : Out.G) if (!std::isfinite(v)) return;
    Out.valid = 1;
}

int fmpc_host_estimator_gain(const double* A_s, int p, int nx, std::vector<double>& G) {
    typedef long double ld;
    std::vector<ld> M((size_t)nx * nx, 0.0L), V((size_t)nx * nx, 0.0L);
    for (int a = 0; a < nx; ++a)
        for (int b = a; b < nx; ++b) {
            ld s = 0.0L;
            for (int i = 0; i < p; ++i) s += (ld)A_s[(size_t)a * p + i] * (ld)A_s[(size_t)b * p + i];
            M[(size_t)a * nx + b] = s; M[(size_t)b * nx + a] = s;
        }
    for (int a = 0; a < nx; ++a) V[(size_t)a * nx + a] = 1.0L;
    for (int sweep = 0; sweep < 60; ++sweep) {
        ld off = 0.0L, dia = 0.0L;
        for (int a = 0; a < nx; ++a) for (int b = 0; b < nx; ++b) { if (a != b) off += M[(size_t)a * nx + b] * M[(size_t)a * nx + b]; else dia += M[(size_t)a * nx + a] * M[(size_t)a * nx + a]; }
        if (off <= 1e-60L * dia || off == 0.0L) break;
        for (int a = 0; a < nx - 1; ++a)
            for (int b = a + 1; b < nx; ++b) {
                const ld apq = M[(size_t)a * nx + b];
                if (apq == 0.0L) continue;
                const ld theta = (M[(size_t)b * nx + b] - M[(size_t)a * nx + a]) / (2.0L * apq);
                const ld t = (theta >= 0.0L ? 1.0L : -1.0L) / (fabsl(theta) + sqrtl(theta * theta + 1.0L));
                const ld c = 1.0L / sqrtl(t * t + 1.0L), s = t * c;
                for (int k = 0; k < nx; ++k) {
                    const ld mka = M[(size_t)k * nx + a], mkb = M[(size_t)k * nx + b];
                    M[(size_t)k * nx + a] = c * mka - s * mkb; M[(size_t)k * nx + b] = s * mka + c * mkb;
                }
                for (int k = 0; k < nx; ++k) {
                    const ld mak = M[(size_t)a * nx + k], mbk = M[(size_t)b * nx + k];
                    M[(size_t)a * nx + k] = c * mak - s * mbk; M[(size_t)b * nx + k] = s * mak + c * mbk;
                }
                for (int k = 0; k < nx; ++k) {
                    const ld vka = V[(size_t)k * nx + a], vkb = V[(size_t)k * nx + b];
                    V[(size_t)k * nx + a] = c * vka - s * vkb; V[(size_t)k * nx + b] = s * vka + c * vkb;
                }
            }
    }
    ld lmax = 0.0L;
    for (int a = 0; a < nx; ++a) lmax = fmaxl(lmax, fabsl(M[(size_t)a * nx + a]));
    const ld tol = (ld)nx * 2.220446049250313e-16L * lmax;
    int rank = 0;
    std::vector<ld> inv(nx, 0.0L);
    for (int a = 0; a < nx; ++a) if (M[(size_t)a * nx + a] > tol) { inv[a] = 1.0L / M[(size_t)a * nx + a]; ++rank; }
    std::vector<ld> Pm((size_t)nx * nx, 0.0L);
    for (int a = 0; a < nx; ++a)
        for (int b = 0; b < nx; ++b) {
            ld s = 0.0L;
            for (int k = 0; k < nx; ++k) s += V[(size_t)a * nx + k] * inv[k] * V[(size_t)b * nx + k];
            Pm[(size_t)a * nx + b] = s;
        }
    G.assign((size_t)nx * p, 0.0);
    for (int a = 0; a < nx; ++a)
        for (int i = 0; i < p; ++i) {
            ld s = 0.0L;
            for (int b = 0; b < nx; ++b) s += Pm[(size_t)a * nx + b] * (ld)A_s[(size_t)b * p + i];
            G[(size_t)a * p + i] = (double)s;
        }
    return rank;
}

void fmpc_host_estimator_dft_images(int len, int d, int first, std::vector<double>& img) {
    typedef long double ld;
    const ld two_pi = 6.283185307179586476925286766559L;
    img.assign((size_t)(len / 4) * 2 * 2 * 64, 0.0);
    for (int y = 0; y < len; ++y)
        for (int j = 0; j < d && j < 32; ++j) {
            const long long e = ((long long)(first + j - len / 2) * (long long)(y - len / 2)) % len;
            const ld ang = -two_pi * (ld)((e + len) % len) / (ld)len;
            const size_t base = (((size_t)(y / 4) * 2 + (j / 16)) * 2) * 64 + (size_t)(y % 4) * 16 + (j % 16);
            img[base] = (double)cosl(ang);
            img[base + 64] = (double)sinl(ang);
        }
}

int fmpc_host_plan_lanes(int nsteps, const unsigned* supersedes, int ngroups, int slots, int tiles_used, int cap, int* lane_of_step, int* wpg_out) {
    if (ngroups < 1) ngroups = 1;
    const int wpg_max = (tiles_used + 3) / 4 > 0 ? (tiles_used + 3) / 4 : 1;
    auto wpg_of = [&](int L) { const int w = slots / (ngroups * L); return w < 1 ? 1 : (w > wpg_max ? wpg_max : w); };
    for (int i = 0; i < nsteps; ++i) lane_of_step[i] = 0;
    *wpg_out = wpg_of(1);
    if (nsteps <= 1) return 1;
    std::vector<int> cls(nsteps), first, len;
    for (int j = 0; j < nsteps; ++j) {
        int rep = j;
        for (int i = 0; i < j; ++i) if (supersedes[j] >> i & 1u) { rep = first[cls[i]]; break; }
        if (rep == j) { cls[j] = (int)first.size(); first.push_back(j); len.push_back(1); }
        else { cls[j] = cls[rep]; ++len[cls[j]]; }
    }
    const int nc = (int)first.size();
    std::vector<int> order(nc);
    for (int c = 0; c < nc; ++c) order[c] = c;
    for (int a = 1; a < nc; ++a)
        for (int b = a; b > 0 && len[order[b]] > len[order[b - 1]]; --b) { const int t = order[b]; order[b] = order[b - 1]; order[b - 1] = t; }
    int Lmax = slots / ngroups < 1 ? 1 : slots / ngroups;
    if (Lmax > nc) Lmax = nc;
    if (cap >= 1 && Lmax > cap) Lmax = cap;
    if (cap < 1) Lmax = 1;
    int bestL = 1; long best = -1;
    std::vector<int> lane_of_cls(nc), best_lanes(nc, 0), load;
    for (int L = 1; L <= Lmax; ++L) {
        load.assign(L, 0);
        for (int o = 0; o < nc; ++o) {
            int to = 0;
            for (int l = 1; l < L; ++l) if (load[l] < load[to]) to = l;
            lane_of_cls[order[o]] = to; load[to] += len[order[o]];
        }
        int H = 0;
        for (int l = 0; l < L; ++l) if (load[l] > H) H = load[l];
        const int w = wpg_of(L), R = (tiles_used + 4 * w - 1) / (4 * w);
        const long cost = (long)H * (R + FMPC_LANE_START_ROUNDS);
        if (best < 0 || cost < best) { best = cost; bestL = L; best_lanes = lane_of_cls; }
    }
    for (int j = 0; j < nsteps; ++j) lane_of_step[j] = best_lanes[cls[j]];
    *wpg_out = wpg_of(bestL);
    return bestL;
}

extern "C" int fmpc_debug_plan_lanes(int nsteps, const unsigned* supersedes, int ngroups, int slots, int tiles_used, int cap, int* lane_of_step,
                                     int* lanes, int* wpg) {
    if (nsteps < 0 || nsteps > 32 || (nsteps && (!supersedes || !lane_of_step)) || !lanes || !wpg) return -1;
    int dummy = 0;
    *lanes = fmpc_host_plan_lanes(nsteps, supersedes, ngroups, slots, tiles_used, cap, nsteps ? lane_of_step : &dummy, wpg);
    return 0;
// ... 87 lines not shown
```

mpc-sensorlessao_amd/csrc/fmpc_host.h:

```cpp
#pragma once
#include <stddef.h>
#include <string.h>
#include <vector>

#include "fmpc_panel_layout.h"

inline double fmpc_host_cm(const double* M, int rows, int r, int c) { return M[(size_t)r + (size_t)c * rows]; }
bool fmpc_host_is_diag(const double* M, int n);
bool fmpc_host_spd_inverse(const std::vector<double>& A, int n, std::vector<double>& inv);

void fmpc_host_add_AXBt(std::vector<double>& out, const std::vector<double>& A, const std::vector<double>& X,
                        const std::vector<double>& B, int n, double sign);

void fmpc_host_y_blocks(int n, int T, bool var2, bool has_xf, const std::vector<double>& a1, const std::vector<double>& a2,
                        const std::vector<double>& X, const std::vector<double>& Xf,
                        std::vector<std::vector<double>>& blocks, std::vector<int>& idxD, std::vector<int>& idx1, std::vector<int>& idx2);

struct FmpcPanelIn {
    int n, m, T, nb, mp, var_order;
    size_t pool_doubles, o_simg, o_limg, o_bt, o_aimg, o_vec, o_ucon, o_dz;
    int limg_cap;
    const double *umax, *umin, *umid, *xmid, *R2, *rl, *Q2, *Qf2, *ql, *qfl, *xf;
    const double *bt;
    const double *a1, *a2;
    const double *blocks;
    const int *idxD, *idx1, *idx2;
};
struct FmpcPanelOut {
    std::vector<double> pool;
    std::vector<int> sched;
    int nsf, nsb, nimg, valid;
    double rp2c, rd2_0;
};
void fmpc_host_panel_layout(int n, int m, int T, int nb, int mp, FmpcPanelIn& L, size_t* o_dump, size_t* total, int* dz_len);
int fmpc_host_build_panel(const FmpcPanelIn& In, double k, FmpcPanelOut& Out);

inline void fmpc_host_key_push(std::vector<double>& key, const double* p, size_t cnt) {
    key.push_back(p ? (double)cnt : -1.0);
    if (p) key.insert(key.end(), p, p + cnt);
}

template <class H>
struct FmpcLru {
    struct Entry { std::vector<double> key; H h; std::vector<double> ramp; unsigned long long stamp; };
    std::vector<Entry> items;
    unsigned long long clock = 0;
    size_t capacity;
    explicit FmpcLru(size_t cap) : capacity(cap) {}
    Entry* find(const std::vector<double>& key) {
        for (Entry& e : items)
            if (e.key.size() == key.size() && memcmp(e.key.data(), key.data(), key.size() * sizeof(double)) == 0) return &e;
        return nullptr;
    }
    template <class D>
    Entry* insert(std::vector<double>&& key, H h, D destroy) {
        if (items.size() >= capacity) {
            size_t old = 0;
            for (size_t i = 1; i < items.size(); ++i) if (items[i].stamp < items[old].stamp) old = i;
            destroy(items[old].h);
            items.erase(items.begin() + old);
        }
        items.push_back(Entry{std::move(key), h, {}, 0});
        return &items.back();
    }
    void touch(Entry* e) { e->stamp = ++clock; }
    template <class D>
    void clear(D destroy) { for (Entry& e : items) destroy(e.h); items.clear(); }
};

#define FMPC_INV_SCALE 1048576.0
bool fmpc_host_inverse_images(int n, int T, int nb, bool var2, int jks, int jks2, const double* a1, const double* a2,
                              const std::vector<double>& nu, std::vector<double>& img, std::vector<double>& nuc,
                              std::vector<double>& jst, std::vector<double>& ncs, std::vector<double>& img2,
                              std::vector<double>& eimg, std::vector<double>& J4, std::vector<double>& nuc4);

#define FM_NC_MAX 108
struct FmpcFirstIn {
    int n, m, T, nb, var2, has_xf;
    const double *bt, *umax, *umin, *umid, *xmid, *R2, *rl, *a1, *a2, *m1, *m2, *xf;
    const double *J;
    const double *nuc;
    double k;
};
struct FmpcFirstOut {
    int nc;
    std::vector<double> K0t, u0c, E, e, Ep, ep;
    std::vector<double> Ec, Epc;
    double e0, ep0, normE, norme, normEp, normep;
};
void fmpc_host_build_first_move(const FmpcFirstIn& In, FmpcFirstOut& Out);

#define FA_KS 14
#define FA_KC (4 * FA_KS)
struct FmpcAffineIn {
    int n, m, T, nb, has_xf, ncJ;
    const double *bt, *umax, *umin, *umid, *xmid, *R2, *rl, *Q2, *Qf2, *ql, *qfl, *a1, *a2;
    const double *J, *nuc;
    double k;
};
#define FA_NU_KS 7
struct FmpcNuStage { int tb, nu, nd, ub; };
#define FMPC_NU_CUT(cnt, p, parts) ((cnt) * (p) / (parts))
struct FmpcAffineOut {
    int rows, tiles;
    int nu_rows, nu_tiles;
    std::vector<double> Kz;
    std::vector<double> img;
    int jbase;
    std::vector<FmpcNuStage> plan;
    std::vector<double> imgG;
};
void fmpc_host_build_affine(const FmpcAffineIn& In, FmpcAffineOut& Out);
void fmpc_host_plan_nu(int m, int n, int T, std::vector<FmpcNuStage>& plan);
int fmpc_host_nu_work(const std::vector<FmpcNuStage>& plan);
int fmpc_host_nu_parts(int T, int work, int W);
int fmpc_host_nu_swap(int T, int parts, int W);
#define FMPC_LANE_START_ROUNDS 3
int fmpc_host_plan_lanes(int nsteps, const unsigned* supersedes, int ngroups, int slots, int tiles_used, int cap, int* lane_of_step, int* wpg);
void fmpc_host_mfma_images(const double* M, int rows, int cols, int ks, std::vector<double>& img);
struct FmpcLoopImages { std::vector<double> imgU, imgE, imgEp, imgB; };
void fmpc_host_build_loop_images(const FmpcFirstOut& O, int n, int m, int ks, bool fused, const double* bt, FmpcLoopImages& out);
void fmpc_host_mfma_a_images(const double* M, int rows, std::vector<double>& img);

struct FmpcRampColdIn {
    int n, m, T, nb, var2, has_xf;
    const double *bt, *a1, *a2;
    const double *umax, *umin, *umid, *xmid, *R2, *rl, *Q2, *Qf2, *ql, *qfl, *xf, *dumin, *dumax;
    double k;
};
struct FmpcRampColdOut {
    int valid;
    std::vector<double> g0;
    std::vector<double> Gf;
    std::vector<double> phib_u, phib_x;
    std::vector<double> gbar_u, gbar_x;
    std::vector<double> hd;
    std::vector<double> erb;
    std::vector<double> cpb;
    std::vector<double> betab;
    std::vector<double> Yinv;
    std::vector<double> G;
    std::vector<double> Xiu0t;
    std::vector<double> y0c;
};
void fmpc_host_build_ramp_cold(const FmpcRampColdIn& In, FmpcRampColdOut& Out);

int fmpc_host_estimator_gain(const double* A_s, int p, int nx, std::vector<double>& G);
void fmpc_host_estimator_dft_images(int len, int d, int first, std::vector<double>& img);
void fmpc_host_estimator_qranges(int len, int ndiv, const double* D_re, const double* D_im, std::vector<int>& qr);

double fmpc_host_mean_square(const double* v, int cnt);
struct fmpc_noise_s;
int fmpc_host_noise_check(const struct fmpc_noise_s* nz, int batch, int sigma_only);

#define FMPC_ZERNIKE_MAXN 14
#define FMPC_ZERNIKE_NCOEF 204
int fmpc_host_zernike_modes(int N, int* n_out, int* m_out);
void fmpc_host_zernike_coefficients(double coef[FMPC_ZERNIKE_NCOEF], unsigned short off[FMPC_ZERNIKE_MAXN + 1][8]);
```

mpc-sensorlessao_amd/csrc/fmpc_kernel_affine.hip:

```cpp
#include <hip/hip_runtime.h>
#include <math.h>
#include <stdlib.h>
#include "fmpc_device.h"
#include "fmpc_affine.h"
#include "../../include/fastmpc.h"

#ifdef FW_TIMING
__device__ unsigned long long fa_trace[1024 * 8];
extern "C" int fmpc_debug_affine_trace(unsigned long long* out) {
    return hipMemcpyFromSymbol(out, HIP_SYMBOL(fa_trace), sizeof(unsigned long long) * 1024 * 8) == hipSuccess ? 0 : -1;
}
#define FA_TICK(k) do { if (tid == 0 && blockIdx.x < 1024) fa_trace[blockIdx.x * 8 + (k)] = (unsigned long long)wall_clock64(); } while (0)
#else
#define FA_TICK(k)
#endif
typedef double d4a __attribute__((ext_vector_type(4)));
typedef double d2a __attribute__((ext_vector_type(2)));
#define FA_MFMA(a, b, c) __builtin_amdgcn_mfma_f64_16x16x4f64((a), (b), (c), 0, 0, 0)
#define FA_THREADS 256
#define FA_CT 4

__device__ __forceinline__ void fa_load_a(double (&A)[FA_KS], const double* img, int tile, int lane) {
    const double* ip = img + (size_t)tile * FA_KS * 64 + lane;
#pragma unroll
    for (int q = 0; q < FA_KS; ++q) A[q] = ip[q * 64];
}

__device__ __forceinline__ void fa_request_a(double (&A)[FA_KS], const double* img, int tile, int lane) {
    const double* ip = img + (size_t)tile * FA_KS * 64 + lane;
    const double* ip2 = ip + 8 * 64;
#define FA_LD(q, base, off) asm volatile("global_load_dwordx2 %0, %1, off offset:" #off : "=v"(A[q]) : "v"(base))
    FA_LD(0, ip, 0); FA_LD(1, ip, 512); FA_LD(2, ip, 1024); FA_LD(3, ip, 1536); FA_LD(4, ip, 2048); FA_LD(5, ip, 2560); FA_LD(6, ip, 3072); FA_LD(7, ip, 3584);
    FA_LD(8, ip2, 0); FA_LD(9, ip2, 512); FA_LD(10, ip2, 1024); FA_LD(11, ip2, 1536); FA_LD(12, ip2, 2048); FA_LD(13, ip2, 2560);
#undef FA_LD
}
template <int BEHIND>
__device__ __forceinline__ void fa_await_a(double (&A)[FA_KS]) {
    asm volatile("s_waitcnt vmcnt(%14)"
                 : "+v"(A[0]), "+v"(A[1]), "+v"(A[2]), "+v"(A[3]), "+v"(A[4]), "+v"(A[5]), "+v"(A[6]), "+v"(A[7]), "+v"(A[8]), "+v"(A[9]),
                   "+v"(A[10]), "+v"(A[11]), "+v"(A[12]), "+v"(A[13])
                 : "n"(BEHIND));
}

__device__ __forceinline__ bool fa_decide(const FaParams& P, double qe, double qp, double rdl, double dn2) {
    const double dn = sqrt(dn2);
    double e2 = qe + P.e0, rp2 = qp + P.ep0;
    const double ce = 4096.0 * 2.220446049250313e-16;
    const double de = ce * (dn2 * P.normE + 2.0 * P.norme * dn + fabs(P.e0));
    const double dp = ce * (dn2 * P.normEp + 2.0 * P.normep * dn + fabs(P.ep0));
    e2 += de;
    rp2 = rp2 - dp > 0.0 ? rp2 - dp : 0.0;
    const double rho2 = rp2 + rdl;
    const bool fin = rp2 < 1e300 && rho2 < 1e300 && e2 < 1e300 && e2 >= 0.0;
    return fin && (rp2 > 4e-16 || rho2 > 4e-12) && e2 <= 0.5 * rho2;
}

template <bool ZOUT, bool NT = false>
__global__ void __launch_bounds__(FA_THREADS, 2) fmpc_cold_affine(FaParams P) {
    __shared__ double sD[FA_KS * FA_CT * 64];
#define FA_SD(ct, cc, k) sD[((((k) >> 2) * FA_CT + (ct)) * 4 + ((k) & 3)) * 16 + (cc)]
    __shared__ double sF[4][3][16];
    const int tid0 = threadIdx.x;
    constexpr int n = FA_N;
    const int wg = (int)blockIdx.x;
    const int ln = wg / P.wgs_per_lane, wl = wg - ln * P.wgs_per_lane;
    const int gi = wl / P.wgs_per_group, slot = wl - gi * P.wgs_per_group;
    const int s_begin = P.lane_begin[ln], s_end = P.lane_begin[ln + 1];
    const int tiles = P.tiles_used, rows = P.rows, m = P.m;
    const int tstep = 4 * P.wgs_per_group;
    { const int tid = tid0; FA_TICK(0); (void)tid; }
    if (wg == 0 && tid0 == 0 && P.handed) *P.handed = 0;
    double A[FA_KS], An[FA_KS];
    const int p0 = gi * FA_CT * 16;
    const int rounds = tiles / tstep;
    const bool forms_wg = P.wgs_per_group >= 8 && rounds >= 2 && slot >= P.wgs_per_group - FA_CT;
    const int nskip = (P.wgs_per_group >= 8 && rounds >= 2) ? 4 * FA_CT : 0;
    const int skip0 = (rounds - 1) * tstep + (P.wgs_per_group - FA_CT) * 4;
    const int tfull = (rounds - (forms_wg ? 1 : 0)) * tstep;
    for (int s = s_begin; s < s_end; ++s) {
    int tid = tid0;
    asm volatile("" : "+v"(tid));
    const int lane = tid & 63, wv = tid >> 6, g = lane >> 4, c = lane & 15;
    double* dump = P.dump + ((blockIdx.x & 15) * FA_THREADS + tid);
    const FaStep& S = P.steps[s];
    const double* const x0_s = S.x0; const double* const x0p_s = S.x0p; const double* const nu0_s = S.nu0;
    double* const zout_s = S.zout; double* const nuout_s = S.nuout; double* const u0out_s = S.u0out;
    int* const status_s = S.status; int* const iters_s = S.iters; double* const step_s = S.step; int* const need_s = S.need;
    int tile = slot * 4 + wv;
    if (s != s_begin) __syncthreads();
    fa_request_a(A, P.img, tile < tiles ? tile : 0, lane);
    {
        const int np = P.batch - p0 < FA_CT * 16 ? P.batch - p0 : FA_CT * 16;
        const double* s0 = x0_s + (size_t)p0 * n;
        const double* s1 = x0p_s ? x0p_s + (size_t)p0 * n : s0;
        double v0[7], v1[7];
#pragma unroll
        for (int j = 0; j < 7; ++j) {
            const int idx = tid + FA_THREADS * j, ic = idx < np * n ? idx : 0;
            v0[j] = s0[ic]; v1[j] = s1[ic];
        }
#pragma unroll
        for (int j = 0; j < 7; ++j) {
            const int idx = tid + FA_THREADS * j;
            if (idx < FA_CT * 16 * n) {
                const int pr = idx / n, k = idx - pr * n;
                const bool on = idx < np * n;
                FA_SD(pr >> 4, pr & 15, k) = on ? v0[j] : 0.0;
                FA_SD(pr >> 4, pr & 15, n + k) = (on && x0p_s) ? v1[j] : 0.0;
            }
        }
        if (tid < FA_CT * 16) { FA_SD(tid >> 4, tid & 15, 2 * n) = 1.0; FA_SD(tid >> 4, tid & 15, 2 * n + 1) = 0.0; }
    }
    __syncthreads();
    FA_TICK(1);
    for (int fct = P.wgs_per_group - 1 - slot; fct < FA_CT; fct += P.wgs_per_group) {
        if (fct < 0 || p0 + fct * 16 >= P.batch) continue;
        const int t = wv;
        double E1[FA_KS], E2[FA_KS], Df[FA_KS];
        fa_load_a(E1, P.imgE, t, lane);
        fa_load_a(E2, P.imgEp, t, lane);
        const int k = 16 * t + c;
        const double le = P.elin[k], lp = P.eplin[k];
        double rdl[4] = {P.rd2_0, P.rd2_0, P.rd2_0, P.rd2_0};
        if (nu0_s && t == 0) {
            double xa[4][2];
#pragma unroll
            for (int r = 0; r < 4; ++r) {
                const int pr = p0 + fct * 16 + 4 * r + g < P.batch ? p0 + fct * 16 + 4 * r + g : P.batch - 1;
                const double* nu = nu0_s + (size_t)pr * P.nb * n;
#pragma unroll
                for (int j = 0; j < 2; ++j) {
                    const int e = c + 16 * j, ec = e < n ? e : 0;
                    xa[r][j] = P.dx0T[ec] + nu[(P.T - 1) * n + ec] + (P.has_xf ? nu[P.T * n + ec] : 0.0);
                }
            }
#pragma unroll
            for (int r = 0; r < 4; ++r) {
                double acc = xa[r][0] * xa[r][0] + (c + 16 < n ? xa[r][1] * xa[r][1] : 0.0);
                acc += __shfl_xor(acc, 1, 64); acc += __shfl_xor(acc, 2, 64); acc += __shfl_xor(acc, 4, 64); acc += __shfl_xor(acc, 8, 64);
                rdl[r] = acc;
            }
        }
#pragma unroll
        for (int q = 0; q < FA_KS; ++q) Df[q] = sD[(q * FA_CT + fct) * 64 + lane];
        d4a ce = {0, 0, 0, 0}, cp = {0, 0, 0, 0};
#pragma unroll
        for (int q = 0; q < FA_KS; ++q) { ce = FA_MFMA(Df[q], E1[q], ce); cp = FA_MFMA(Df[q], E2[q], cp); }
        double qe[4], qp[4], dn2[4];
#pragma unroll
        for (int r = 0; r < 4; ++r) {
            const double dv = k < 2 * n ? FA_SD(fct, 4 * r + g, k < 2 * n ? k : 0) : 0.0;
            qe[r] = dv * (ce[r] + le); qp[r] = dv * (cp[r] + lp); dn2[r] = dv * dv;
#pragma unroll
            for (int o = 1; o < 16; o <<= 1) { qe[r] += __shfl_xor(qe[r], o, 64); qp[r] += __shfl_xor(qp[r], o, 64); dn2[r] += __shfl_xor(dn2[r], o, 64); }
            if (c == 0) { sF[t][0][4 * r + g] = qe[r]; sF[t][1][4 * r + g] = qp[r]; sF[t][2][4 * r + g] = dn2[r]; }
        }
        __syncthreads();
        if (t == 0 && c == 0) {
#pragma unroll
            for (int r = 0; r < 4; ++r) {
                const int i = 4 * r + g, pp = p0 + fct * 16 + i;
                if (pp < P.batch) {
                    const double se = (sF[0][0][i] + sF[1][0][i]) + (sF[2][0][i] + sF[3][0][i]);
                    const double sp = (sF[0][1][i] + sF[1][1][i]) + (sF[2][1][i] + sF[3][1][i]);
                    const double sn = (sF[0][2][i] + sF[1][2][i]) + (sF[2][2][i] + sF[3][2][i]);
                    const bool clear = fa_decide(P, se, sp, rdl[r], sn);
                    need_s[pp] = clear ? 0 : 1;
                    if (!clear && P.nflag) atomicAdd(P.nflag, 1);
                    if (clear) {
                        if (status_s) status_s[pp] = FMPC_OK;
                        if (iters_s) iters_s[pp] = 1;
                        if (step_s) for (int q = 0; q < P.step_ld; ++q) step_s[(size_t)pp * P.step_ld + q] = q == 0 ? 1.0 : -1.0;
                    }
                }
            }
        }
        __syncthreads();
    }
    {
        const int wg_w = slot * 4 + wv;
        const int nleft = nskip + (tiles - rounds * tstep);
        for (int task = wg_w; task < nleft * FA_CT; task += tstep) {
            const int j = task / FA_CT, ct = task % FA_CT;
            const int lt = j < nskip ? skip0 + j : rounds * tstep + (j - nskip);
            double Al[FA_KS], Dl[FA_KS];
            fa_load_a(Al, P.img, lt, lane);
#pragma unroll
            for (int q = 0; q < FA_KS; ++q) Dl[q] = sD[(q * FA_CT + ct) * 64 + lane];
            d4a acc = {0, 0, 0, 0};
#pragma unroll
            for (int q = 0; q < FA_KS; ++q) acc = FA_MFMA(Dl[q], Al[q], acc);
            const int row = 16 * lt + c;
#pragma unroll
            for (int r = 0; r < 4; ++r) {
                const int pp = (gi * FA_CT + ct) * 16 + 4 * r + g;
                if (ZOUT && lt < P.tiles && row < rows && pp < P.batch) zout_s[(size_t)pp * P.ldz + row] = acc[r];
                if (ZOUT && lt >= P.tiles && row - 16 * P.tiles < P.nu_rows && pp < P.batch) nuout_s[(size_t)pp * P.nu_rows + (row - 16 * P.tiles)] = acc[r];
                if (u0out_s != nullptr && row < m && pp < P.batch) u0out_s[(size_t)pp * m + row] = acc[r];
            }
        }
    }
    if (tile >= tfull) { fa_await_a<0>(A); continue; }
    double D[FA_CT][FA_KS];
#pragma unroll
    for (int ct = 0; ct < FA_CT; ++ct)
#pragma unroll
        for (int q = 0; q < FA_KS; ++q) D[ct][q] = sD[(q * FA_CT + ct) * 64 + lane];
    FA_TICK(4);
    fa_await_a<0>(A);
    FA_TICK(5);
    for (; tile < tfull; tile += tstep) {
        const int nxt = tile + tstep < tfull ? tile + tstep : tile;
        fa_request_a(An, P.img, nxt, lane);
        d4a acc[FA_CT];
#pragma unroll
        for (int ct = 0; ct < FA_CT; ++ct) acc[ct] = (d4a){0, 0, 0, 0};
#pragma unroll
        for (int q = 0; q < FA_KS; ++q)
#pragma unroll
            for (int ct = 0; ct < FA_CT; ++ct) acc[ct] = FA_MFMA(D[ct][q], A[q], acc[ct]);
        const int row = 16 * tile + c;
        if (ZOUT) {
            const bool isnu = tile >= P.tiles;
            const int rloc = isnu ? row - 16 * P.tiles : row, rcnt = isnu ? P.nu_rows : rows, ld = isnu ? P.nu_rows : P.ldz;
            double* obase = isnu ? nuout_s : zout_s;
            const unsigned voz = (unsigned)(g * ld + rloc);
            const bool rok = rloc < rcnt;
#pragma unroll
            for (int ct = 0; ct < FA_CT; ++ct)
#pragma unroll
                for (int r = 0; r < 4; ++r) {
                    const int pb = (gi * FA_CT + ct) * 16 + 4 * r;
                    double* zb = obase + (size_t)pb * ld + voz;
                    double* dst = (rok && pb + g < P.batch) ? zb : dump;
                    if (NT) __builtin_nontemporal_store(acc[ct][r], dst);
                    else *dst = acc[ct][r];
                }
        }
        if (!ZOUT || (u0out_s != nullptr && 16 * tile < m)) {
            const unsigned vou = (unsigned)(g * m + row);
            const bool rok = row < m;
#pragma unroll
            for (int ct = 0; ct < FA_CT; ++ct)
#pragma unroll
                for (int r = 0; r < 4; ++r) {
                    const int pb = (gi * FA_CT + ct) * 16 + 4 * r;
                    double* ub = u0out_s + (size_t)pb * m + vou;
                    double* dst = (rok && pb + g < P.batch) ? ub : dump;
                    *dst = acc[ct][r];
                }
        }
#ifdef FW_TIMING
        if (tile == slot * 4 + wv) { asm volatile("s_nop 0" :: "v"(acc[0][0]), "v"(acc[1][0]), "v"(acc[2][0]), "v"(acc[3][0])); FA_TICK(6); }
#endif
        fa_await_a<16>(An);
#pragma unroll
        for (int q = 0; q < FA_KS; ++q) A[q] = An[q];
#ifdef FW_TIMING
        if (tile == slot * 4 + wv) FA_TICK(2);
#endif
    }
    FA_TICK(3);
    }
}

hipError_t fmpc_launch_affine(FaParams P, int num_cu, hipStream_t stream, const unsigned* supersedes) {
    if (P.n != 27 || 2 * P.n + 2 > FA_KC || 7 * FA_THREADS < FA_CT * 16 * P.n) return hipErrorInvalidValue;
    if (P.nsteps < 0 || P.nsteps > FMPC_STRETCH_MAX) return hipErrorInvalidValue;
    if (P.nsteps == 0) {
        P.nsteps = 1;
        P.steps[0] = {P.x0, P.x0p, P.nu0, P.zout, P.nuout, P.u0out, P.status, P.iters, P.step, P.need};
    }
    P.x0 = P.steps[0].x0; P.zout = P.steps[0].zout; P.nuout = P.steps[0].nuout; P.u0out = P.steps[0].u0out;
    bool aligned = true;
    for (int s = 0; s < P.nsteps; ++s) {
        const FaStep& S = P.steps[s];
        if (!S.x0 || !S.need || (S.zout == nullptr) != (P.zout == nullptr) || (S.nuout == nullptr) != (P.nuout == nullptr) ||
            (S.u0out == nullptr) != (P.u0out == nullptr)) return hipErrorInvalidValue;
        aligned = aligned && ((size_t)S.zout & 127) == 0;
    }
    if (!P.zout && !P.u0out) return hipErrorInvalidValue;
    const int ncol = (P.batch + 15) / 16, ngroups = (ncol + FA_CT - 1) / FA_CT;
    P.tiles_used = P.zout ? P.tiles + (P.nuout ? P.nu_tiles : 0) : (P.m + 15) / 16;
    if (P.ldz < P.rows) P.ldz = P.rows;
    static const bool no_nt = [] { const char* e = getenv("FMPC_AFFINE_NO_NT"); return e && e[0] == '1'; }();
    const bool nt = P.zout && !no_nt && P.ldz % 16 == 0 && aligned;
    int cap = FMPC_STRETCH_LANES_DEFAULT;
    if (P.nsteps > 1) { const char* e = getenv("FMPC_STRETCH_LANES"); if (e && e[0]) cap = atoi(e); }
    if (cap < 1 || !supersedes) cap = 1;
    int lane_of[FMPC_STRETCH_MAX], wpg = 1;
    P.nlanes = fmpc_host_plan_lanes(P.nsteps, supersedes, ngroups, 2 * num_cu, P.tiles_used, cap, lane_of, &wpg);
    P.wgs_per_group = wpg;
    P.wgs_per_lane = ngroups * wpg;
    {
        FaStep in_chain_order[FMPC_STRETCH_MAX];
        for (int s = 0; s < P.nsteps; ++s) in_chain_order[s] = P.steps[s];
        int k = 0;
        for (int l = 0; l < P.nlanes; ++l) {
            P.lane_begin[l] = k;
            for (int s = 0; s < P.nsteps; ++s) if (lane_of[s] == l) P.steps[k++] = in_chain_order[s];
        }
        for (int l = P.nlanes; l <= FMPC_STRETCH_MAX; ++l) P.lane_begin[l] = k;
    }
    const int grid = P.nlanes * ngroups * wpg;
    if (P.zout && P.imgG) {
        const char* e = getenv("FMPC_AFFINE_DIRECT");
        if (!(e && e[0] == '1')) return fmpc_launch_affine_nu(P, grid, nt, stream);
    }
    if (P.zout && nt) hipLaunchKernelGGL((fmpc_cold_affine<true, true>), dim3(grid), dim3(FA_THREADS), 0, stream, P);
    else if (P.zout) hipLaunchKernelGGL((fmpc_cold_affine<true, false>), dim3(grid), dim3(FA_THREADS), 0, stream, P);
    else hipLaunchKernelGGL((fmpc_cold_affine<false, false>), dim3(grid), dim3(FA_THREADS), 0, stream, P);
    return hipGetLastError();
}
```

mpc-sensorlessao_amd/csrc/fmpc_kernel_affine_nu.hip:

```cpp
#include <hip/hip_runtime.h>
#include <math.h>
#include <stdlib.h>
#include "fmpc_affine_dev.h"

#ifdef FW_TIMING
__device__ unsigned long long fa_nu_trace[1024 * 8];
extern "C" int fmpc_debug_affine_nu_trace(unsigned long long* out) {
    return hipMemcpyFromSymbol(out, HIP_SYMBOL(fa_nu_trace), sizeof(unsigned long long) * 1024 * 8) == hipSuccess ? 0 : -1;
}
#define FA_TICK(k) do { if (tid == 0 && blockIdx.x < 1024) fa_nu_trace[blockIdx.x * 8 + (k)] = (unsigned long long)wall_clock64(); } while (0)
#else
#define FA_TICK(k)
#endif

typedef __attribute__((address_space(1))) double fa_gdouble;
__device__ __forceinline__ fa_gdouble* fa_pick(bool ok, double* a, double* b) {
    unsigned long long mk = 0ull - (unsigned long long)ok;
    asm volatile("" : "+v"(mk));
    return (fa_gdouble*)(((unsigned long long)a & mk) | ((unsigned long long)b & ~mk));
}

template <bool NT, bool FULL>
__device__ __forceinline__ void fa_nu_store(const FaParams& P, const d4a (&acc)[FA_CT], int tile, int gi, int lane,
                                            double* zout_s, double* nuout_s, double* dump) {
    asm volatile("" : "+v"(lane));
    const int g = lane >> 4, c = lane & 15;
    const bool isnu = !FULL && tile >= P.tiles;
    const int r0 = isnu ? 16 * (tile - P.tiles) : 16 * tile, rcnt = isnu ? P.nu_rows : P.rows, ld = isnu ? P.nu_rows : P.ldz;
    double* obase = (isnu ? nuout_s : zout_s) + (size_t)(gi * FA_CT * 16) * ld + r0;
    const unsigned voz = (unsigned)(g * ld + c);
    const bool rok = r0 + c < rcnt;
#pragma unroll
    for (int ct = 0; ct < FA_CT; ++ct)
#pragma unroll
        for (int r = 0; r < 4; ++r) {
            const int pb = (gi * FA_CT + ct) * 16 + 4 * r;
            double* zb = obase + (size_t)((ct * 16 + 4 * r) * ld) + voz;
            fa_gdouble* dst = FULL ? (fa_gdouble*)zb : fa_pick(rok && pb + g < P.batch, zb, dump);
            if (NT) __builtin_nontemporal_store(acc[ct][r], dst);
            else *dst = acc[ct][r];
            if (!FULL) __builtin_amdgcn_sched_barrier(0);
        }
}

template <bool NT, bool FULL>
__device__ __forceinline__ void fa_nu_utiles(const FaParams& P, double (&A)[FA_NU_KS], const d4a (&n0)[FA_CT], const d4a (&n1)[FA_CT],
                                             int ub, int ue, int ui, int gi, int lane, double* zout_s, double* dump) {
    double An[FA_NU_KS];
    int tile = ub;
    do {
        fa_request_g(An, P.imgG, ui + (tile + 1 < ue ? tile + 1 : tile) - ub, lane);
        d4a acc[FA_CT];
#pragma unroll
        for (int ct = 0; ct < FA_CT; ++ct) acc[ct] = (d4a){0, 0, 0, 0};
#pragma unroll
        for (int q = 0; q < FA_NU_KS; ++q)
#pragma unroll
            for (int ct = 0; ct < FA_CT; ++ct) acc[ct] = FA_MFMA(q < 4 ? n0[ct][q & 3] : n1[ct][q & 3], A[q], acc[ct]);
        fa_nu_store<NT, FULL>(P, acc, tile, gi, lane, zout_s, nullptr, dump);
        fa_await_g<16>(An);
#pragma unroll
        for (int q = 0; q < FA_NU_KS; ++q) A[q] = An[q];
    } while (++tile < ue);
}

template <bool NT, bool U0>
__device__ __forceinline__ void fa_nu_direct(const FaParams& P, double (&A)[FA_KS], double (&An)[FA_KS], const double (&D)[FA_CT][FA_KS],
                                             int db, int de, int after, int gi, int lane, double* zout_s, double* nuout_s, double* u0out_s, double* dump) {
    const int m = P.m;
    int tile = db;
    do {
        if (!U0) fa_request_a(An, P.img, tile + 1 < de ? tile + 1 : after, lane);
        d4a acc[FA_CT];
#pragma unroll
        for (int ct = 0; ct < FA_CT; ++ct) acc[ct] = (d4a){0, 0, 0, 0};
#pragma unroll
        for (int q = 0; q < FA_KS; ++q)
#pragma unroll
            for (int ct = 0; ct < FA_CT; ++ct) acc[ct] = FA_MFMA(D[ct][q], A[q], acc[ct]);
        if (U0) {
            asm volatile("" :: "v"(acc[0][0]), "v"(acc[1][0]), "v"(acc[2][0]), "v"(acc[3][0]));
            fa_request_a(A, P.img, tile + 1 < de ? tile + 1 : after, lane);
        }
        fa_nu_store<NT, false>(P, acc, tile, gi, lane, zout_s, nuout_s, dump);
        if (U0) {
            int lu = lane;
            asm volatile("" : "+v"(lu));
            const int g = lu >> 4, c = lu & 15;
            const int row = 16 * tile + c;
            const unsigned vou = (unsigned)(g * m + row);
            const bool rok = row < m;
#pragma unroll
            for (int ct = 0; ct < FA_CT; ++ct)
#pragma unroll
                for (int r = 0; r < 4; ++r) {
                    const int pb = (gi * FA_CT + ct) * 16 + 4 * r;
                    double* ubp = u0out_s + (size_t)pb * m + vou;
                    fa_gdouble* dst = fa_pick(rok && pb + g < P.batch, ubp, dump);
                    *dst = acc[ct][r];
                    __builtin_amdgcn_sched_barrier(0);
                }
        }
        if (U0) fa_await_a<32>(A);
        else {
            fa_await_a<16>(An);
#pragma unroll
            for (int q = 0; q < FA_KS; ++q) A[q] = An[q];
        }
    } while (++tile < de);
}

struct FaNuItem { int ub, ue, ui, db, de, jt; };
__device__ __forceinline__ FaNuItem fa_nu_item(const FaParams& P, int it) {
    FaNuItem I = {0, 0, 0, 0, 0, -1};
    const int nst = P.T * P.nparts;
    if (it < nst) {
        const int js = it / P.nparts, part = it - js * P.nparts;
        const int j = js == P.swap ? 0 : (js == 0 ? P.swap : js);
        const int tb = P.plan[4 * j], nu = P.plan[4 * j + 1], nd = P.plan[4 * j + 2], u0 = FMPC_NU_CUT(nu, part, P.nparts);
        I.ub = tb + u0; I.ue = tb + FMPC_NU_CUT(nu, part + 1, P.nparts); I.ui = P.plan[4 * j + 3] + u0;
        I.db = tb + nu + FMPC_NU_CUT(nd, part, P.nparts); I.de = tb + nu + FMPC_NU_CUT(nd, part + 1, P.nparts);
        if (I.ue > I.ub) I.jt = P.jbase + 2 * (j - 1);
    } else {
        I.db = P.tiles + 4 * (it - nst);
        I.de = I.db + 4 < P.tiles + P.nu_tiles ? I.db + 4 : P.tiles + P.nu_tiles;
    }
    return I;
}

template <bool NT>
__global__ void __launch_bounds__(FA_THREADS, 2) fmpc_cold_nu(FaParams P) {
    __shared__ double sD[FA_KS * FA_CT * 64];
    __shared__ double sF[4][3][16];
    const int tid0 = threadIdx.x;
    const int wg = (int)blockIdx.x;
    const int ln = wg / P.wgs_per_lane, wl = wg - ln * P.wgs_per_lane;
    const int gi = wl / P.wgs_per_group, slot = wl - gi * P.wgs_per_group;
    const int s_begin = P.lane_begin[ln], s_end = P.lane_begin[ln + 1];
    const int nwav = 4 * P.wgs_per_group;
    { const int tid = tid0; FA_TICK(0); (void)tid; }
    if (wg == 0 && tid0 == 0 && P.handed) *P.handed = 0;
    const int p0 = gi * FA_CT * 16;
    for (int s = s_begin; s < s_end; ++s) {
    int tid = tid0;
    asm volatile("" : "+v"(tid));
    const int wv = __builtin_amdgcn_readfirstlane(tid >> 6);
    const FaStep& S = P.steps[s];
    const double* const x0_s = S.x0; const double* const x0p_s = S.x0p; const double* const nu0_s = S.nu0;
    double* const zout_s = S.zout; double* const nuout_s = S.nuout; double* const u0out_s = S.u0out;
    int* const status_s = S.status; int* const iters_s = S.iters; double* const step_s = S.step; int* const need_s = S.need;
    if (s != s_begin) __syncthreads();
    fa_stage(sD, P, x0_s, x0p_s, p0, tid);
    __syncthreads();
    FA_TICK(1);
    fa_forms(sD, sF, P, slot, wv, tid & 63, p0, nu0_s, need_s, status_s, iters_s, step_s);
    FA_TICK(2);
    for (int it = slot * 4 + wv; it < P.nitems; it += nwav) {
        int lane = tid & 63;
        asm volatile("" : "+v"(lane));
        const FaNuItem I = fa_nu_item(P, it);
        if (I.de <= I.db && I.jt < 0) continue;
        double A[FA_KS], An[FA_KS];
        fa_request_a(A, P.img, I.de > I.db ? I.db : I.jt, lane);
        double* dump = P.dump + ((blockIdx.x & 15) * FA_THREADS + wv * 64 + lane);
        const int ub = I.ub, ue = I.ue, ui = I.ui, db = I.db, de = I.de, jt = I.jt;
        double D[FA_CT][FA_KS];
#pragma unroll
        for (int ct = 0; ct < FA_CT; ++ct)
#pragma unroll
            for (int q = 0; q < FA_KS; ++q) D[ct][q] = sD[(q * FA_CT + ct) * 64 + lane];
        fa_await_a<0>(A);
        if (de > db) {
            const int after = jt >= 0 ? jt : db;
            if (u0out_s != nullptr && 16 * db < P.m) fa_nu_direct<NT, true>(P, A, An, D, db, de, after, gi, lane, zout_s, nuout_s, u0out_s, dump);
            else fa_nu_direct<NT, false>(P, A, An, D, db, de, after, gi, lane, zout_s, nuout_s, u0out_s, dump);
        }
#ifdef FW_TIMING
        if (it == slot * 4 + wv) FA_TICK(4);
#endif
        if (jt < 0) continue;
        d4a n0[FA_CT], n1[FA_CT];
        double G[FA_NU_KS];
        fa_request_a(An, P.img, jt + 1, lane);
        fa_request_g(G, P.imgG, ui, lane);
#pragma unroll
        for (int ct = 0; ct < FA_CT; ++ct) { n0[ct] = (d4a){0, 0, 0, 0}; n1[ct] = (d4a){0, 0, 0, 0}; }
#pragma unroll
        for (int q = 0; q < FA_KS; ++q) n0[0] = FA_MFMA(A[q], D[0][q], n0[0]);
        fa_await_a<FA_NU_KS>(An);
#pragma unroll
        for (int q = 0; q < FA_KS; ++q) n1[0] = FA_MFMA(An[q], D[0][q], n1[0]);
#pragma unroll
        for (int ct = 1; ct < FA_CT; ++ct)
#pragma unroll
            for (int q = 0; q < FA_KS; ++q) { n0[ct] = FA_MFMA(A[q], D[ct][q], n0[ct]); n1[ct] = FA_MFMA(An[q], D[ct][q], n1[ct]); }
        fa_await_g<0>(G);
#ifdef FW_TIMING
        if (it == slot * 4 + wv) { asm volatile("s_nop 0" :: "v"(n1[0][0]), "v"(n1[1][0]), "v"(n1[2][0]), "v"(n1[3][0])); FA_TICK(5); }
#endif
        if ((gi + 1) * FA_CT * 16 <= P.batch) fa_nu_utiles<NT, true>(P, G, n0, n1, ub, ue, ui, gi, lane, zout_s, dump);
        else fa_nu_utiles<NT, false>(P, G, n0, n1, ub, ue, ui, gi, lane, zout_s, dump);
#ifdef FW_TIMING
        if (it == slot * 4 + wv) FA_TICK(6);
#endif
    }
    FA_TICK(3);
    }
}

hipError_t fmpc_launch_affine_nu(FaParams P, int grid, bool nt, hipStream_t stream) {
    if (P.n != FA_N || !P.zout || !P.imgG || !P.plan || P.nu_work <= 0 || grid < 1) return hipErrorInvalidValue;
    P.nparts = fmpc_host_nu_parts(P.T, P.nu_work, 4 * P.wgs_per_group);
    P.swap = fmpc_host_nu_swap(P.T, P.nparts, 4 * P.wgs_per_group);
    P.nitems = P.T * P.nparts + (P.nuout ? (P.nu_tiles + 3) / 4 : 0);
    if (nt) hipLaunchKernelGGL((fmpc_cold_nu<true>), dim3(grid), dim3(FA_THREADS), 0, stream, P);
    else hipLaunchKernelGGL((fmpc_cold_nu<false>), dim3(grid), dim3(FA_THREADS), 0, stream, P);
    return hipGetLastError();
}
```

Measured before the change: 94.38 million.

## Balance nu-kernel work across waves with host-precomputed deal tables

Builds host-side per-wave work tables that greedily move individual direct tiles from the most loaded wave to the least loaded one, then makes the cold nu kernel walk its own contiguous slice of dealt items instead of striding over the formula-derived item list. The aim is to even out per-wave load so the kernel's tail is set by a balanced maximum rather than by the unluckiest wave. It adds an indirect tile-id load per tile and extra table memory in the pool. The old formula path is kept as a fallback for large groups or when FMPC_AFFINE_DEAL=0.

```diff
diff --git a/mpc-sensorlessao_amd/csrc/fmpc_affine.h b/mpc-sensorlessao_amd/csrc/fmpc_affine.h
--- a/mpc-sensorlessao_amd/csrc/fmpc_affine.h
+++ b/mpc-sensorlessao_amd/csrc/fmpc_affine.h
@@ -34,8 +34,11 @@
     const int* plan;
     int jbase, nu_work;
     int nparts, nitems, swap;
+    const int* deal_all;
+    const int* deal;
 };
 
 #define FMPC_STRETCH_LANES_DEFAULT FMPC_STRETCH_MAX
 hipError_t fmpc_launch_affine(FaParams P, int num_cu, hipStream_t stream, const unsigned* supersedes = nullptr);
 hipError_t fmpc_launch_affine_nu(FaParams P, int grid, bool nt, hipStream_t stream);
+hipError_t fmpc_launch_affine_nu_formula(FaParams P, int grid, bool nt, hipStream_t stream);
diff --git a/mpc-sensorlessao_amd/csrc/fmpc_affine_nu_dev.h b/mpc-sensorlessao_amd/csrc/fmpc_affine_nu_dev.h
--- /dev/null
+++ b/mpc-sensorlessao_amd/csrc/fmpc_affine_nu_dev.h
@@ -0,0 +1,234 @@
+#pragma once
+#include <hip/hip_runtime.h>
+#include <math.h>
+#include <stdlib.h>
+#include "fmpc_affine_dev.h"
+
+#ifdef FW_TIMING
+static __device__ unsigned long long fa_nu_trace[1024 * 12];
+extern "C" int FA_NU_TRACE_EXPORT(unsigned long long* out) {
+    return hipMemcpyFromSymbol(out, HIP_SYMBOL(fa_nu_trace), sizeof(unsigned long long) * 1024 * 12) == hipSuccess ? 0 : -1;
+}
+#define FA_TICK(k) do { if (tid == 0 && blockIdx.x < 1024) fa_nu_trace[blockIdx.x * 8 + (k)] = (unsigned long long)wall_clock64(); } while (0)
+#define FA_TICK_WAVE(wv) do { if ((tid & 63) == 0 && blockIdx.x < 1024) fa_nu_trace[1024 * 8 + blockIdx.x * 4 + (wv)] = (unsigned long long)wall_clock64(); } while (0)
+#else
+#define FA_TICK(k)
+#define FA_TICK_WAVE(wv)
+#endif
+
+typedef __attribute__((address_space(1))) double fa_gdouble;
+__device__ __forceinline__ fa_gdouble* fa_pick(bool ok, double* a, double* b) {
+    unsigned long long mk = 0ull - (unsigned long long)ok;
+    asm volatile("" : "+v"(mk));
+    return (fa_gdouble*)(((unsigned long long)a & mk) | ((unsigned long long)b & ~mk));
+}
+
+template <bool NT, bool FULL>
+__device__ __forceinline__ void fa_nu_store(const FaParams& P, const d4a (&acc)[FA_CT], int tile, int gi, int lane,
+                                            double* zout_s, double* nuout_s, double* dump) {
+    asm volatile("" : "+v"(lane));
+    const int g = lane >> 4, c = lane & 15;
+    const bool isnu = !FULL && tile >= P.tiles;
+    const int r0 = isnu ? 16 * (tile - P.tiles) : 16 * tile, rcnt = isnu ? P.nu_rows : P.rows, ld = isnu ? P.nu_rows : P.ldz;
+    double* obase = (isnu ? nuout_s : zout_s) + (size_t)(gi * FA_CT * 16) * ld + r0;
+    const unsigned voz = (unsigned)(g * ld + c);
+    const bool rok = r0 + c < rcnt;
+#pragma unroll
+    for (int ct = 0; ct < FA_CT; ++ct)
+#pragma unroll
+        for (int r = 0; r < 4; ++r) {
+            const int pb = (gi * FA_CT + ct) * 16 + 4 * r;
+            double* zb = obase + (size_t)((ct * 16 + 4 * r) * ld) + voz;
+            fa_gdouble* dst = FULL ? (fa_gdouble*)zb : fa_pick(rok && pb + g < P.batch, zb, dump);
+            if (NT) __builtin_nontemporal_store(acc[ct][r], dst);
+            else *dst = acc[ct][r];
+            if (!FULL) __builtin_amdgcn_sched_barrier(0);
+        }
+}
+
+template <bool NT, bool FULL>
+__device__ __forceinline__ void fa_nu_utiles(const FaParams& P, double (&A)[FA_NU_KS], const d4a (&n0)[FA_CT], const d4a (&n1)[FA_CT],
+                                             int ub, int ue, int ui, int gi, int lane, double* zout_s, double* dump) {
+    double An[FA_NU_KS];
+    int tile = ub;
+    do {
+        fa_request_g(An, P.imgG, ui + (tile + 1 < ue ? tile + 1 : tile) - ub, lane);
+        d4a acc[FA_CT];
+#pragma unroll
+        for (int ct = 0; ct < FA_CT; ++ct) acc[ct] = (d4a){0, 0, 0, 0};
+#pragma unroll
+        for (int q = 0; q < FA_NU_KS; ++q)
+#pragma unroll
+            for (int ct = 0; ct < FA_CT; ++ct) acc[ct] = FA_MFMA(q < 4 ? n0[ct][q & 3] : n1[ct][q & 3], A[q], acc[ct]);
+        fa_nu_store<NT, FULL>(P, acc, tile, gi, lane, zout_s, nullptr, dump);
+        fa_await_g<16>(An);
+#pragma unroll
+        for (int q = 0; q < FA_NU_KS; ++q) A[q] = An[q];
+    } while (++tile < ue);
+}
+
+template <bool DEAL>
+__device__ __forceinline__ int fa_nu_id(const int* ids, int i) { return DEAL ? ids[i] : i; }
+template <bool NT, bool U0, bool DEAL>
+__device__ __forceinline__ void fa_nu_direct(const FaParams& P, double (&A)[FA_KS], double (&An)[FA_KS], const double (&D)[FA_CT][FA_KS],
+                                             const int* ids, int db, int de, int tile, int after, int gi, int lane, double* zout_s, double* nuout_s,
+                                             double* u0out_s, double* dump) {
+    const int m = P.m;
+    int i = db;
+    const int id1 = fa_nu_id<DEAL>(ids, db + 1 < de ? db + 1 : db);
+    int next = db + 1 < de ? id1 : after;
+    do {
+        const int id2 = fa_nu_id<DEAL>(ids, i + 2 < de ? i + 2 : i);
+        if (!U0) fa_request_a(An, P.img, next, lane);
+        d4a acc[FA_CT];
+#pragma unroll
+        for (int ct = 0; ct < FA_CT; ++ct) acc[ct] = (d4a){0, 0, 0, 0};
+#pragma unroll
+        for (int q = 0; q < FA_KS; ++q)
+#pragma unroll
+            for (int ct = 0; ct < FA_CT; ++ct) acc[ct] = FA_MFMA(D[ct][q], A[q], acc[ct]);
+        if (U0) {
+            asm volatile("" :: "v"(acc[0][0]), "v"(acc[1][0]), "v"(acc[2][0]), "v"(acc[3][0]));
+            fa_request_a(A, P.img, next, lane);
+        }
+        fa_nu_store<NT, false>(P, acc, tile, gi, lane, zout_s, nuout_s, dump);
+        if (U0) {
+            int lu = lane;
+            asm volatile("" : "+v"(lu));
+            const int g = lu >> 4, c = lu & 15;
+            const int row = 16 * tile + c;
+            const unsigned vou = (unsigned)(g * m + row);
+            const bool rok = row < m;
+#pragma unroll
+            for (int ct = 0; ct < FA_CT; ++ct)
+#pragma unroll
+                for (int r = 0; r < 4; ++r) {
+                    const int pb = (gi * FA_CT + ct) * 16 + 4 * r;
+                    double* ubp = u0out_s + (size_t)pb * m + vou;
+                    fa_gdouble* dst = fa_pick(rok && pb + g < P.batch, ubp, dump);
+                    *dst = acc[ct][r];
+                    __builtin_amdgcn_sched_barrier(0);
+                }
+        }
+        if (U0) fa_await_a<32>(A);
+        else {
+            fa_await_a<16>(An);
+#pragma unroll
+            for (int q = 0; q < FA_KS; ++q) A[q] = An[q];
+        }
+        tile = next;
+        next = i + 2 < de ? id2 : after;
+    } while (++i < de);
+}
+
+struct FaNuItem { int ub, ue, ui, db, de, jt; };
+__device__ __forceinline__ FaNuItem fa_nu_item_dealt(const FaParams& P, const int* dl, int nwav, int it) {
+    const int* e = dl + (nwav + 1) + 6 * it;
+    FaNuItem I = {e[1], e[2], e[3], e[4], e[5], e[0] >= 0 ? P.jbase + e[0] : -1};
+    return I;
+}
+__device__ __forceinline__ FaNuItem fa_nu_item(const FaParams& P, int it) {
+    FaNuItem I = {0, 0, 0, 0, 0, -1};
+    const int nst = P.T * P.nparts;
+    if (it < nst) {
+        const int js = it / P.nparts, part = it - js * P.nparts;
+        const int j = js == P.swap ? 0 : (js == 0 ? P.swap : js);
+        const int tb = P.plan[4 * j], nu = P.plan[4 * j + 1], nd = P.plan[4 * j + 2], u0 = FMPC_NU_CUT(nu, part, P.nparts);
+        I.ub = tb + u0; I.ue = tb + FMPC_NU_CUT(nu, part + 1, P.nparts); I.ui = P.plan[4 * j + 3] + u0;
+        I.db = tb + nu + FMPC_NU_CUT(nd, part, P.nparts); I.de = tb + nu + FMPC_NU_CUT(nd, part + 1, P.nparts);
+        if (I.ue > I.ub) I.jt = P.jbase + 2 * (j - 1);
+    } else {
+        I.db = P.tiles + 4 * (it - nst);
+        I.de = I.db + 4 < P.tiles + P.nu_tiles ? I.db + 4 : P.tiles + P.nu_tiles;
+    }
+    return I;
+}
+
+template <bool NT, bool DEAL>
+__global__ void __launch_bounds__(FA_THREADS, 2) fmpc_cold_nu(FaParams P) {
+    __shared__ double sD[FA_KS * FA_CT * 64];
+    __shared__ double sF[4][3][16];
+    const int tid0 = threadIdx.x;
+    const int wg = (int)blockIdx.x;
+    const int ln = wg / P.wgs_per_lane, wl = wg - ln * P.wgs_per_lane;
+    const int gi = wl / P.wgs_per_group, slot = wl - gi * P.wgs_per_group;
+    const int s_begin = P.lane_begin[ln], s_end = P.lane_begin[ln + 1];
+    const int nwav = 4 * P.wgs_per_group;
+    { const int tid = tid0; FA_TICK(0); (void)tid; }
+    if (wg == 0 && tid0 == 0 && P.handed) *P.handed = 0;
+    const int p0 = gi * FA_CT * 16;
+    for (int s = s_begin; s < s_end; ++s) {
+    int tid = tid0;
+    asm volatile("" : "+v"(tid));
+    const int wv = __builtin_amdgcn_readfirstlane(tid >> 6);
+    const FaStep& S = P.steps[s];
+    const double* const x0_s = S.x0; const double* const x0p_s = S.x0p; const double* const nu0_s = S.nu0;
+    double* const zout_s = S.zout; double* const nuout_s = S.nuout; double* const u0out_s = S.u0out;
+    int* const status_s = S.status; int* const iters_s = S.iters; double* const step_s = S.step; int* const need_s = S.need;
+    if (s != s_begin) __syncthreads();
+#ifdef FW_TIMING
+    if (s == s_begin + 3) FA_TICK(7);
+#endif
+    fa_stage(sD, P, x0_s, x0p_s, p0, tid);
+    __syncthreads();
+    FA_TICK(1);
+    fa_forms(sD, sF, P, slot, wv, tid & 63, p0, nu0_s, need_s, status_s, iters_s, step_s);
+    FA_TICK(2);
+    const int* const dl = DEAL ? P.deal_all + *P.deal : nullptr;
+    const int it_first = DEAL ? dl[slot * 4 + wv] : slot * 4 + wv, it_end = DEAL ? dl[slot * 4 + wv + 1] : P.nitems, it_step = DEAL ? 1 : nwav;
+    for (int it = it_first; it < it_end; it += it_step) {
+        int lane = tid & 63;
+        asm volatile("" : "+v"(lane));
+        const FaNuItem I = DEAL ? fa_nu_item_dealt(P, dl, nwav, it) : fa_nu_item(P, it);
+        if (I.de <= I.db && I.jt < 0) continue;
+        double A[FA_KS], An[FA_KS];
+        const int ub = I.ub, ue = I.ue, ui = I.ui, db = I.db, de = I.de, jt = I.jt;
+        const int tile0 = fa_nu_id<DEAL>(dl, db);
+        fa_request_a(A, P.img, de > db ? tile0 : jt, lane);
+        double* dump = P.dump + ((blockIdx.x & 15) * FA_THREADS + wv * 64 + lane);
+        double D[FA_CT][FA_KS];
+#pragma unroll
+        for (int ct = 0; ct < FA_CT; ++ct)
+#pragma unroll
+            for (int q = 0; q < FA_KS; ++q) D[ct][q] = sD[(q * FA_CT + ct) * 64 + lane];
+        fa_await_a<0>(A);
+        if (de > db) {
+            const int after = jt >= 0 ? jt : tile0;
+            if (u0out_s != nullptr && 16 * tile0 < P.m) fa_nu_direct<NT, true, DEAL>(P, A, An, D, dl, db, de, tile0, after, gi, lane, zout_s, nuout_s, u0out_s, dump);
+            else fa_nu_direct<NT, false, DEAL>(P, A, An, D, dl, db, de, tile0, after, gi, lane, zout_s, nuout_s, u0out_s, dump);
+        }
+#ifdef FW_TIMING
+        if (it == it_first) FA_TICK(4);
+#endif
+        if (jt < 0) continue;
+        d4a n0[FA_CT], n1[FA_CT];
+        double G[FA_NU_KS];
+        fa_request_a(An, P.img, jt + 1, lane);
+        fa_request_g(G, P.imgG, ui, lane);
+#pragma unroll
+        for (int ct = 0; ct < FA_CT; ++ct) { n0[ct] = (d4a){0, 0, 0, 0}; n1[ct] = (d4a){0, 0, 0, 0}; }
+#pragma unroll
+        for (int q = 0; q < FA_KS; ++q) n0[0] = FA_MFMA(A[q], D[0][q], n0[0]);
+        fa_await_a<FA_NU_KS>(An);
+#pragma unroll
+        for (int q = 0; q < FA_KS; ++q) n1[0] = FA_MFMA(An[q], D[0][q], n1[0]);
+#pragma unroll
+        for (int ct = 1; ct < FA_CT; ++ct)
+#pragma unroll
+            for (int q = 0; q < FA_KS; ++q) { n0[ct] = FA_MFMA(A[q], D[ct][q], n0[ct]); n1[ct] = FA_MFMA(An[q], D[ct][q], n1[ct]); }
+        fa_await_g<0>(G);
+#ifdef FW_TIMING
+        if (it == it_first) { asm volatile("s_nop 0" :: "v"(n1[0][0]), "v"(n1[1][0]), "v"(n1[2][0]), "v"(n1[3][0])); FA_TICK(5); }
+#endif
+        if ((gi + 1) * FA_CT * 16 <= P.batch) fa_nu_utiles<NT, true>(P, G, n0, n1, ub, ue, ui, gi, lane, zout_s, dump);
+        else fa_nu_utiles<NT, false>(P, G, n0, n1, ub, ue, ui, gi, lane, zout_s, dump);
+#ifdef FW_TIMING
+        if (it == it_first) FA_TICK(6);
+#endif
+    }
+#ifdef FW_TIMING
+    if (s == s_begin + 2) FA_TICK_WAVE(wv);
+#endif
+    FA_TICK(3);
+    }
+}
diff --git a/mpc-sensorlessao_amd/csrc/fmpc_api.hip b/mpc-sensorlessao_amd/csrc/fmpc_api.hip
--- a/mpc-sensorlessao_amd/csrc/fmpc_api.hip
+++ b/mpc-sensorlessao_amd/csrc/fmpc_api.hip
@@ -929,7 +929,7 @@
     const size_t oK = push(O.K0t), ou = push(O.u0c), oE = push(O.Ec), oe = push(O.e), oEp = push(O.Epc), oep = push(O.ep), om = push(m12t), od = push(dx0T);
     h->fa_valid = 0;
     FmpcAffineOut AO;
-    size_t oA = 0, oAE = 0, oAEp = 0, oAl = 0, oAlp = 0, oAd = 0, oAG = 0, oAP = 0;
+    size_t oA = 0, oAE = 0, oAEp = 0, oAl = 0, oAlp = 0, oAd = 0, oAG = 0, oAP = 0, oAT = 0;
     bool fa_ok = !h->fa_disabled && 2 * n + 2 <= FA_KC;
     if (fa_ok) {
         FmpcAffineIn AI;
@@ -955,6 +955,11 @@
             std::vector<double> planw((AO.plan.size() * sizeof(FmpcNuStage) + sizeof(double) - 1) / sizeof(double), 0.0);
             memcpy(planw.data(), AO.plan.data(), AO.plan.size() * sizeof(FmpcNuStage));
             oAG = push(AO.imgG); oAP = push(planw);
+            std::vector<int> deal;
+            fmpc_host_nu_deal_tables(AO.plan, T, AO.nu_tiles, deal);
+            std::vector<double> dealw((deal.size() * sizeof(int) + sizeof(double) - 1) / sizeof(double), 0.0);
+            memcpy(dealw.data(), deal.data(), deal.size() * sizeof(int));
+            oAT = push(dealw);
         }
     }
     h->fl_valid = 0; h->fs_valid = 0;
@@ -987,6 +992,7 @@
         A.img = h->fm_pool + oA; A.imgE = h->fm_pool + oAE; A.imgEp = h->fm_pool + oAEp; A.elin = h->fm_pool + oAl; A.eplin = h->fm_pool + oAlp; A.dump = h->fm_pool + oAd;
         if (!AO.imgG.empty()) {
             A.imgG = h->fm_pool + oAG; A.plan = (const int*)(h->fm_pool + oAP); A.jbase = AO.jbase; A.nu_work = fmpc_host_nu_work(AO.plan);
+            A.deal_all = (const int*)(h->fm_pool + oAT);
         }
         A.dx0T = P.dx0T; A.e0 = O.e0; A.ep0 = O.ep0; A.normE = O.normE; A.norme = O.norme; A.normEp = O.normEp; A.normep = O.normep; A.rd2_0 = h->pn_rd2_0;
         h->fa_valid = 1;
diff --git a/mpc-sensorlessao_amd/csrc/fmpc_host.cpp b/mpc-sensorlessao_amd/csrc/fmpc_host.cpp
--- a/mpc-sensorlessao_amd/csrc/fmpc_host.cpp
+++ b/mpc-sensorlessao_amd/csrc/fmpc_host.cpp
@@ -918,6 +918,97 @@
     return parts == 1 && W >= 1 && T > W - 1 && T % W != 0 ? W - 1 : 0;
 }
 
+namespace {
+struct NuDealItem { int jt, ub, ue, ui; std::vector<int> d; bool keep; };
+int nu_deal_load(const std::vector<NuDealItem>& L) {
+    int w = 0;
+    for (const NuDealItem& I : L) w += 7 * (I.ue - I.ub) + 14 * (int)I.d.size() + (I.ue > I.ub ? 28 : 0);
+    return w;
+}
+bool nu_deal_move(std::vector<std::vector<NuDealItem>>& Wv, int* maxload) {
+    const int W = (int)Wv.size();
+    std::vector<int> load(W);
+    int mx = 0, lo = 0;
+    for (int w = 0; w < W; ++w) { load[w] = nu_deal_load(Wv[w]); if (load[w] > mx) mx = load[w]; if (load[w] < load[lo]) lo = w; }
+    *maxload = mx;
+    for (int h = 0; h < W; ++h) {
+        if (load[h] != mx || h == lo) continue;
+        for (int k = (int)Wv[h].size() - 1; k >= 0; --k) {
+            NuDealItem& I = Wv[h][k];
+            if (I.keep || I.d.empty()) continue;
+            if (load[lo] + 14 >= load[h]) return false;
+            const int id = I.d.back();
+            I.d.pop_back();
+            if (!Wv[lo].empty() && !Wv[lo].back().keep) Wv[lo].back().d.push_back(id);
+            else Wv[lo].push_back(NuDealItem{-1, 0, 0, 0, std::vector<int>(1, id), false});
+            return true;
+        }
+    }
+    return false;
+}
+void nu_deal_start(const std::vector<FmpcNuStage>& plan, int T, int W, int nu_out_tiles, std::vector<std::vector<NuDealItem>>& Wv) {
+    const int parts = fmpc_host_nu_parts(T, fmpc_host_nu_work(plan), W), swap = fmpc_host_nu_swap(T, parts, W);
+    const int nst = T * parts, nitems = nst + (nu_out_tiles + 3) / 4;
+    const int tiles = plan[T - 1].tb + plan[T - 1].nu + plan[T - 1].nd;
+    Wv.assign(W, std::vector<NuDealItem>());
+    for (int it = 0; it < nitems; ++it) {
+        NuDealItem I{-1, 0, 0, 0, std::vector<int>(), false};
+        if (it < nst) {
+            const int js = it / parts, part = it - js * parts;
+            const int j = js == swap ? 0 : (js == 0 ? swap : js);
+            const FmpcNuStage& S = plan[j];
+            const int u0 = FMPC_NU_CUT(S.nu, part, parts);
+            I.ub = S.tb + u0; I.ue = S.tb + FMPC_NU_CUT(S.nu, part + 1, parts); I.ui = S.ub + u0;
+            for (int t = S.tb + S.nu + FMPC_NU_CUT(S.nd, part, parts); t < S.tb + S.nu + FMPC_NU_CUT(S.nd, part + 1, parts); ++t) I.d.push_back(t);
+            if (I.ue > I.ub) I.jt = 2 * (j - 1);
+            else I.ub = I.ue = I.ui = 0;
+            I.keep = j == 0;
+        } else
+            for (int t = tiles + 4 * (it - nst); t < tiles + 4 * (it - nst) + 4 && t < tiles + nu_out_tiles; ++t) I.d.push_back(t);
+        Wv[it % W].push_back(I);
+    }
+}
+}
+
+void fmpc_host_nu_deal(const std::vector<FmpcNuStage>& plan, int T, int W, int nu_out_tiles, FmpcNuDeal& out) {
+    out.wave.assign(W > 0 ? W + 1 : 1, 0); out.items.clear(); out.ids.clear();
+    if (T < 1 || W < 1 || (int)plan.size() < T) return;
+    if (nu_out_tiles < 0) nu_out_tiles = 0;
+    std::vector<std::vector<NuDealItem>> Wv;
+    nu_deal_start(plan, T, W, nu_out_tiles, Wv);
+    std::vector<int> before;
+    int mx = 0;
+    while (nu_deal_move(Wv, &mx)) before.push_back(mx);
+    size_t moves = 0;
+    while (moves < before.size() && before[moves] > mx) ++moves;
+    nu_deal_start(plan, T, W, nu_out_tiles, Wv);
+    for (size_t k = 0; k < moves; ++k) nu_deal_move(Wv, &mx);
+    for (int w = 0; w < W; ++w) {
+        out.wave[w] = (int)out.items.size();
+        for (const NuDealItem& I : Wv[w]) {
+            if (I.ue <= I.ub && I.d.empty()) continue;
+            out.items.push_back(FmpcNuDealItem{I.jt, I.ub, I.ue, I.ui, (int)out.ids.size(), (int)(out.ids.size() + I.d.size())});
+            out.ids.insert(out.ids.end(), I.d.begin(), I.d.end());
+        }
+    }
+    out.wave[W] = (int)out.items.size();
+}
+
+void fmpc_host_nu_deal_tables(const std::vector<FmpcNuStage>& plan, int T, int nu_tiles, std::vector<int>& blob) {
+    blob.assign(2 * FMPC_NU_DEAL_WPG, 0);
+    if (T < 1 || (int)plan.size() < T) return;
+    for (int wpg = 1; wpg <= FMPC_NU_DEAL_WPG; ++wpg)
+        for (int nu = 0; nu < 2; ++nu) {
+            FmpcNuDeal D;
+            fmpc_host_nu_deal(plan, T, 4 * wpg, nu ? nu_tiles : 0, D);
+            const int base = (int)blob.size(), off = (int)D.wave.size() + 6 * (int)D.items.size();
+            blob[2 * (wpg - 1) + nu] = base;
+            blob.insert(blob.end(), D.wave.begin(), D.wave.end());
+            for (const FmpcNuDealItem& I : D.items) { const int v[6] = {I.jt, I.ub, I.ue, I.ui, off + I.d0, off + I.d1}; blob.insert(blob.end(), v, v + 6); }
+            blob.insert(blob.end(), D.ids.begin(), D.ids.end());
+        }
+}
+
 extern "C" int fmpc_debug_plan_nu(int m, int n, int T, int W, int* plan4, int* parts, int* swap) {
     if (m < 1 || n < 1 || T < 1 || !plan4) return -1;
     std::vector<FmpcNuStage> plan;
@@ -932,6 +1023,23 @@
     if (cnt < 0 || parts < 1 || p < 0 || p >= parts || !b || !e) return -1;
     *b = FMPC_NU_CUT(cnt, p, parts); *e = FMPC_NU_CUT(cnt, p + 1, parts);
     return 0;
+}
+extern "C" int fmpc_debug_nu_deal(int m, int n, int T, int W, int nu_out_tiles, int* wave, int* items, int cap_items, int* ids, int cap_ids, int* nids) {
+    if (m < 1 || n < 1 || T < 1 || W < 1 || nu_out_tiles < 0 || !wave || !items || !ids || !nids) return -1;
+    std::vector<FmpcNuStage> plan;
+    fmpc_host_plan_nu(m, n, T, plan);
+    FmpcNuDeal D;
+    fmpc_host_nu_deal(plan, T, W, nu_out_tiles, D);
+    if ((int)D.items.size() > cap_items || (int)D.ids.size() > cap_ids) return -2;
+    std::copy(D.wave.begin(), D.wave.end(), wave);
+    for (size_t k = 0; k < D.items.size(); ++k) {
+        const FmpcNuDealItem& I = D.items[k];
+        const int v[6] = {I.jt, I.ub, I.ue, I.ui, I.d0, I.d1};
+        std::copy(v, v + 6, items + 6 * k);
+    }
+    std::copy(D.ids.begin(), D.ids.end(), ids);
+    *nids = (int)D.ids.size();
+    return (int)D.items.size();
 }
 extern "C" int fmpc_debug_build_affine_nu(int n, int m, int T, int nb, int has_xf, double k, const double* const* arr, double* Kz, double* imgJ, double* imgG) {
     if (n != 27 || m < 1 || T < 1 || nb < T || !arr) return -1;
diff --git a/mpc-sensorlessao_amd/csrc/fmpc_host.h b/mpc-sensorlessao_amd/csrc/fmpc_host.h
--- a/mpc-sensorlessao_amd/csrc/fmpc_host.h
+++ b/mpc-sensorlessao_amd/csrc/fmpc_host.h
@@ -115,6 +115,15 @@
 int fmpc_host_nu_work(const std::vector<FmpcNuStage>& plan);
 int fmpc_host_nu_parts(int T, int work, int W);
 int fmpc_host_nu_swap(int T, int parts, int W);
+struct FmpcNuDealItem { int jt, ub, ue, ui, d0, d1; };
+struct FmpcNuDeal {
+    std::vector<int> wave;
+    std::vector<FmpcNuDealItem> items;
+    std::vector<int> ids;
+};
+void fmpc_host_nu_deal(const std::vector<FmpcNuStage>& plan, int T, int W, int nu_out_tiles, FmpcNuDeal& out);
+#define FMPC_NU_DEAL_WPG 16
+void fmpc_host_nu_deal_tables(const std::vector<FmpcNuStage>& plan, int T, int nu_tiles, std::vector<int>& blob);
 #define FMPC_LANE_START_ROUNDS 3
 int fmpc_host_plan_lanes(int nsteps, const unsigned* supersedes, int ngroups, int slots, int tiles_used, int cap, int* lane_of_step, int* wpg);
 void fmpc_host_mfma_images(const double* M, int rows, int cols, int ks, std::vector<double>& img);
diff --git a/mpc-sensorlessao_amd/csrc/fmpc_kernel_affine.hip b/mpc-sensorlessao_amd/csrc/fmpc_kernel_affine.hip
--- a/mpc-sensorlessao_amd/csrc/fmpc_kernel_affine.hip
+++ b/mpc-sensorlessao_amd/csrc/fmpc_kernel_affine.hip
@@ -290,6 +290,7 @@
     if (cap < 1 || !supersedes) cap = 1;
     int lane_of[FMPC_STRETCH_MAX], wpg = 1;
     P.nlanes = fmpc_host_plan_lanes(P.nsteps, supersedes, ngroups, 2 * num_cu, P.tiles_used, cap, lane_of, &wpg);
+    { const char* e = getenv("FMPC_AFFINE_WPG_MAX"); if (e && e[0]) { const int k = atoi(e); if (k >= 1 && k < wpg) wpg = k; } }
     P.wgs_per_group = wpg;
     P.wgs_per_lane = ngroups * wpg;
     {
diff --git a/mpc-sensorlessao_amd/csrc/fmpc_kernel_affine_nu.hip b/mpc-sensorlessao_amd/csrc/fmpc_kernel_affine_nu.hip
--- a/mpc-sensorlessao_amd/csrc/fmpc_kernel_affine_nu.hip
+++ b/mpc-sensorlessao_amd/csrc/fmpc_kernel_affine_nu.hip
@@ -1,219 +1,12 @@
-#include <hip/hip_runtime.h>
-#include <math.h>
-#include <stdlib.h>
-#include "fmpc_affine_dev.h"
-
-#ifdef FW_TIMING
-__device__ unsigned long long fa_nu_trace[1024 * 8];
-extern "C" int fmpc_debug_affine_nu_trace(unsigned long long* out) {
-    return hipMemcpyFromSymbol(out, HIP_SYMBOL(fa_nu_trace), sizeof(unsigned long long) * 1024 * 8) == hipSuccess ? 0 : -1;
-}
-#define FA_TICK(k) do { if (tid == 0 && blockIdx.x < 1024) fa_nu_trace[blockIdx.x * 8 + (k)] = (unsigned long long)wall_clock64(); } while (0)
-#else
-#define FA_TICK(k)
-#endif
-
-typedef __attribute__((address_space(1))) double fa_gdouble;
-__device__ __forceinline__ fa_gdouble* fa_pick(bool ok, double* a, double* b) {
-    unsigned long long mk = 0ull - (unsigned long long)ok;
-    asm volatile("" : "+v"(mk));
-    return (fa_gdouble*)(((unsigned long long)a & mk) | ((unsigned long long)b & ~mk));
-}
-
-template <bool NT, bool FULL>
-__device__ __forceinline__ void fa_nu_store(const FaParams& P, const d4a (&acc)[FA_CT], int tile, int gi, int lane,
-                                            double* zout_s, double* nuout_s, double* dump) {
-    asm volatile("" : "+v"(lane));
-    const int g = lane >> 4, c = lane & 15;
-    const bool isnu = !FULL && tile >= P.tiles;
-    const int r0 = isnu ? 16 * (tile - P.tiles) : 16 * tile, rcnt = isnu ? P.nu_rows : P.rows, ld = isnu ? P.nu_rows : P.ldz;
-    double* obase = (isnu ? nuout_s : zout_s) + (size_t)(gi * FA_CT * 16) * ld + r0;
-    const unsigned voz = (unsigned)(g * ld + c);
-    const bool rok = r0 + c < rcnt;
-#pragma unroll
-    for (int ct = 0; ct < FA_CT; ++ct)
-#pragma unroll
-        for (int r = 0; r < 4; ++r) {
-            const int pb = (gi * FA_CT + ct) * 16 + 4 * r;
-            double* zb = obase + (size_t)((ct * 16 + 4 * r) * ld) + voz;
-            fa_gdouble* dst = FULL ? (fa_gdouble*)zb : fa_pick(rok && pb + g < P.batch, zb, dump);
-            if (NT) __builtin_nontemporal_store(acc[ct][r], dst);
-            else *dst = acc[ct][r];
-            if (!FULL) __builtin_amdgcn_sched_barrier(0);
-        }
-}
-
-template <bool NT, bool FULL>
-__device__ __forceinline__ void fa_nu_utiles(const FaParams& P, double (&A)[FA_NU_KS], const d4a (&n0)[FA_CT], const d4a (&n1)[FA_CT],
-                                             int ub, int ue, int ui, int gi, int lane, double* zout_s, double* dump) {
-    double An[FA_NU_KS];
-    int tile = ub;
-    do {
-        fa_request_g(An, P.imgG, ui + (tile + 1 < ue ? tile + 1 : tile) - ub, lane);
-        d4a acc[FA_CT];
-#pragma unroll
-        for (int ct = 0; ct < FA_CT; ++ct) acc[ct] = (d4a){0, 0, 0, 0};
-#pragma unroll
-        for (int q = 0; q < FA_NU_KS; ++q)
-#pragma unroll
-            for (int ct = 0; ct < FA_CT; ++ct) acc[ct] = FA_MFMA(q < 4 ? n0[ct][q & 3] : n1[ct][q & 3], A[q], acc[ct]);
-        fa_nu_store<NT, FULL>(P, acc, tile, gi, lane, zout_s, nullptr, dump);
-        fa_await_g<16>(An);
-#pragma unroll
-        for (int q = 0; q < FA_NU_KS; ++q) A[q] = An[q];
-    } while (++tile < ue);
-}
-
-template <bool NT, bool U0>
-__device__ __forceinline__ void fa_nu_direct(const FaParams& P, double (&A)[FA_KS], double (&An)[FA_KS], const double (&D)[FA_CT][FA_KS],
-                                             int db, int de, int after, int gi, int lane, double* zout_s, double* nuout_s, double* u0out_s, double* dump) {
-    const int m = P.m;
-    int tile = db;
-    do {
-        if (!U0) fa_request_a(An, P.img, tile + 1 < de ? tile + 1 : after, lane);
-        d4a acc[FA_CT];
-#pragma unroll
-        for (int ct = 0; ct < FA_CT; ++ct) acc[ct] = (d4a){0, 0, 0, 0};
-#pragma unroll
-        for (int q = 0; q < FA_KS; ++q)
-#pragma unroll
-            for (int ct = 0; ct < FA_CT; ++ct) acc[ct] = FA_MFMA(D[ct][q], A[q], acc[ct]);
-        if (U0) {
-            asm volatile("" :: "v"(acc[0][0]), "v"(acc[1][0]), "v"(acc[2][0]), "v"(acc[3][0]));
-            fa_request_a(A, P.img, tile + 1 < de ? tile + 1 : after, lane);
-        }
-        fa_nu_store<NT, false>(P, acc, tile, gi, lane, zout_s, nuout_s, dump);
-        if (U0) {
-            int lu = lane;
-            asm volatile("" : "+v"(lu));
-            const int g = lu >> 4, c = lu & 15;
-            const int row = 16 * tile + c;
-            const unsigned vou = (unsigned)(g * m + row);
-            const bool rok = row < m;
-#pragma unroll
-            for (int ct = 0; ct < FA_CT; ++ct)
-#pragma unroll
-                for (int r = 0; r < 4; ++r) {
-                    const int pb = (gi * FA_CT + ct) * 16 + 4 * r;
-                    double* ubp = u0out_s + (size_t)pb * m + vou;
-                    fa_gdouble* dst = fa_pick(rok && pb + g < P.batch, ubp, dump);
-                    *dst = acc[ct][r];
-                    __builtin_amdgcn_sched_barrier(0);
-                }
-        }
-        if (U0) fa_await_a<32>(A);
-        else {
-            fa_await_a<16>(An);
-#pragma unroll
-            for (int q = 0; q < FA_KS; ++q) A[q] = An[q];
-        }
-    } while (++tile < de);
-}
-
-struct FaNuItem { int ub, ue, ui, db, de, jt; };
-__device__ __forceinline__ FaNuItem fa_nu_item(const FaParams& P, int it) {
-    FaNuItem I = {0, 0, 0, 0, 0, -1};
-    const int nst = P.T * P.nparts;
-    if (it < nst) {
-        const int js = it / P.nparts, part = it - js * P.nparts;
-        const int j = js == P.swap ? 0 : (js == 0 ? P.swap : js);
-        const int tb = P.plan[4 * j], nu = P.plan[4 * j + 1], nd = P.plan[4 * j + 2], u0 = FMPC_NU_CUT(nu, part, P.nparts);
-        I.ub = tb + u0; I.ue = tb + FMPC_NU_CUT(nu, part + 1, P.nparts); I.ui = P.plan[4 * j + 3] + u0;
-        I.db = tb + nu + FMPC_NU_CUT(nd, part, P.nparts); I.de = tb + nu + FMPC_NU_CUT(nd, part + 1, P.nparts);
-        if (I.ue > I.ub) I.jt = P.jbase + 2 * (j - 1);
-    } else {
-        I.db = P.tiles + 4 * (it - nst);
-        I.de = I.db + 4 < P.tiles + P.nu_tiles ? I.db + 4 : P.tiles + P.nu_tiles;
-    }
-    return I;
-}
-
-template <bool NT>
-__global__ void __launch_bounds__(FA_THREADS, 2) fmpc_cold_nu(FaParams P) {
-    __shared__ double sD[FA_KS * FA_CT * 64];
-    __shared__ double sF[4][3][16];
-    const int tid0 = threadIdx.x;
-    const int wg = (int)blockIdx.x;
-    const int ln = wg / P.wgs_per_lane, wl = wg - ln * P.wgs_per_lane;
-    const int gi = wl / P.wgs_per_group, slot = wl - gi * P.wgs_per_group;
-    const int s_begin = P.lane_begin[ln], s_end = P.lane_begin[ln + 1];
-    const int nwav = 4 * P.wgs_per_group;
-    { const int tid = tid0; FA_TICK(0); (void)tid; }
-    if (wg == 0 && tid0 == 0 && P.handed) *P.handed = 0;
-    const int p0 = gi * FA_CT * 16;
-    for (int s = s_begin; s < s_end; ++s) {
-    int tid = tid0;
-    asm volatile("" : "+v"(tid));
-    const int wv = __builtin_amdgcn_readfirstlane(tid >> 6);
-    const FaStep& S = P.steps[s];
-    const double* const x0_s = S.x0; const double* const x0p_s = S.x0p; const double* const nu0_s = S.nu0;
-    double* const zout_s = S.zout; double* const nuout_s = S.nuout; double* const u0out_s = S.u0out;
-    int* const status_s = S.status; int* const iters_s = S.iters; double* const step_s = S.step; int* const need_s = S.need;
-    if (s != s_begin) __syncthreads();
-    fa_stage(sD, P, x0_s, x0p_s, p0, tid);
-    __syncthreads();
-    FA_TICK(1);
-    fa_forms(sD, sF, P, slot, wv, tid & 63, p0, nu0_s, need_s, status_s, iters_s, step_s);
-    FA_TICK(2);
-    for (int it = slot * 4 + wv; it < P.nitems; it += nwav) {
-        int lane = tid & 63;
-        asm volatile("" : "+v"(lane));
-        const FaNuItem I = fa_nu_item(P, it);
-        if (I.de <= I.db && I.jt < 0) continue;
-        double A[FA_KS], An[FA_KS];
-        fa_request_a(A, P.img, I.de > I.db ? I.db : I.jt, lane);
-        double* dump = P.dump + ((blockIdx.x & 15) * FA_THREADS + wv * 64 + lane);
-        const int ub = I.ub, ue = I.ue, ui = I.ui, db = I.db, de = I.de, jt = I.jt;
-        double D[FA_CT][FA_KS];
-#pragma unroll
-        for (int ct = 0; ct < FA_CT; ++ct)
-#pragma unroll
-            for (int q = 0; q < FA_KS; ++q) D[ct][q] = sD[(q * FA_CT + ct) * 64 + lane];
-        fa_await_a<0>(A);
-        if (de > db) {
-            const int after = jt >= 0 ? jt : db;
-            if (u0out_s != nullptr && 16 * db < P.m) fa_nu_direct<NT, true>(P, A, An, D, db, de, after, gi, lane, zout_s, nuout_s, u0out_s, dump);
-            else fa_nu_direct<NT, false>(P, A, An, D, db, de, after, gi, lane, zout_s, nuout_s, u0out_s, dump);
-        }
-#ifdef FW_TIMING
-        if (it == slot * 4 + wv) FA_TICK(4);
-#endif
-        if (jt < 0) continue;
-        d4a n0[FA_CT], n1[FA_CT];
-        double G[FA_NU_KS];
-        fa_request_a(An, P.img, jt + 1, lane);
-        fa_request_g(G, P.imgG, ui, lane);
-#pragma unroll
-        for (int ct = 0; ct < FA_CT; ++ct) { n0[ct] = (d4a){0, 0, 0, 0}; n1[ct] = (d4a){0, 0, 0, 0}; }
-#pragma unroll
-        for (int q = 0; q < FA_KS; ++q) n0[0] = FA_MFMA(A[q], D[0][q], n0[0]);
-        fa_await_a<FA_NU_KS>(An);
-#pragma unroll
-        for (int q = 0; q < FA_KS; ++q) n1[0] = FA_MFMA(An[q], D[0][q], n1[0]);
-#pragma unroll
-        for (int ct = 1; ct < FA_CT; ++ct)
-#pragma unroll
-            for (int q = 0; q < FA_KS; ++q) { n0[ct] = FA_MFMA(A[q], D[ct][q], n0[ct]); n1[ct] = FA_MFMA(An[q], D[ct][q], n1[ct]); }
-        fa_await_g<0>(G);
-#ifdef FW_TIMING
-        if (it == slot * 4 + wv) { asm volatile("s_nop 0" :: "v"(n1[0][0]), "v"(n1[1][0]), "v"(n1[2][0]), "v"(n1[3][0])); FA_TICK(5); }
-#endif
-        if ((gi + 1) * FA_CT * 16 <= P.batch) fa_nu_utiles<NT, true>(P, G, n0, n1, ub, ue, ui, gi, lane, zout_s, dump);
-        else fa_nu_utiles<NT, false>(P, G, n0, n1, ub, ue, ui, gi, lane, zout_s, dump);
-#ifdef FW_TIMING
-        if (it == slot * 4 + wv) FA_TICK(6);
-#endif
-    }
-    FA_TICK(3);
-    }
-}
+#define FA_NU_TRACE_EXPORT fmpc_debug_affine_nu_trace
+#include "fmpc_affine_nu_dev.h"
 
 hipError_t fmpc_launch_affine_nu(FaParams P, int grid, bool nt, hipStream_t stream) {
-    if (P.n != FA_N || !P.zout || !P.imgG || !P.plan || P.nu_work <= 0 || grid < 1) return hipErrorInvalidValue;
-    P.nparts = fmpc_host_nu_parts(P.T, P.nu_work, 4 * P.wgs_per_group);
-    P.swap = fmpc_host_nu_swap(P.T, P.nparts, 4 * P.wgs_per_group);
-    P.nitems = P.T * P.nparts + (P.nuout ? (P.nu_tiles + 3) / 4 : 0);
-    if (nt) hipLaunchKernelGGL((fmpc_cold_nu<true>), dim3(grid), dim3(FA_THREADS), 0, stream, P);
-    else hipLaunchKernelGGL((fmpc_cold_nu<false>), dim3(grid), dim3(FA_THREADS), 0, stream, P);
+    if (P.n != FA_N || !P.zout || !P.imgG || !P.plan || !P.deal_all || P.nu_work <= 0 || grid < 1) return hipErrorInvalidValue;
+    const char* e = getenv("FMPC_AFFINE_DEAL");
+    if (P.wgs_per_group > FMPC_NU_DEAL_WPG || (e && e[0] == '0')) return fmpc_launch_affine_nu_formula(P, grid, nt, stream);
+    P.deal = P.deal_all + 2 * (P.wgs_per_group - 1) + (P.nuout ? 1 : 0);
+    if (nt) hipLaunchKernelGGL((fmpc_cold_nu<true, true>), dim3(grid), dim3(FA_THREADS), 0, stream, P);
+    else hipLaunchKernelGGL((fmpc_cold_nu<false, true>), dim3(grid), dim3(FA_THREADS), 0, stream, P);
     return hipGetLastError();
 }
diff --git a/mpc-sensorlessao_amd/csrc/fmpc_kernel_affine_nu_formula.hip b/mpc-sensorlessao_amd/csrc/fmpc_kernel_affine_nu_formula.hip
--- /dev/null
+++ b/mpc-sensorlessao_amd/csrc/fmpc_kernel_affine_nu_formula.hip
@@ -0,0 +1,13 @@
+#define FA_NU_TRACE_EXPORT fmpc_debug_affine_nu_formula_trace
+#include "fmpc_affine_nu_dev.h"
+
+hipError_t fmpc_launch_affine_nu_formula(FaParams P, int grid, bool nt, hipStream_t stream) {
+    if (P.n != FA_N || !P.zout || !P.imgG || !P.plan || P.nu_work <= 0 || grid < 1) return hipErrorInvalidValue;
+    P.nparts = fmpc_host_nu_parts(P.T, P.nu_work, 4 * P.wgs_per_group);
+    P.swap = fmpc_host_nu_swap(P.T, P.nparts, 4 * P.wgs_per_group);
+    P.nitems = P.T * P.nparts + (P.nuout ? (P.nu_tiles + 3) / 4 : 0);
+    P.deal = nullptr;
+    if (nt) hipLaunchKernelGGL((fmpc_cold_nu<true, false>), dim3(grid), dim3(FA_THREADS), 0, stream, P);
+    else hipLaunchKernelGGL((fmpc_cold_nu<false, false>), dim3(grid), dim3(FA_THREADS), 0, stream, P);
+    return hipGetLastError();
+}
```

Result: no change. 93.93 million, median of 2 (-0.5%).
